# pflanze/LAPIS-SILO

Hardware: AMD Instinct MI355X
Metric: Mutations-scan positions*sequences/s (higher is better)
Workload: dtype u64; 1 GPU; 10000000-sequence x 29903-nt nucleotide Mutations scan (minProportion 0.05) with a PangoLineage sublineage filter (B.1*), through QueryEngine::executeQuery; sequences=10000000, positions=29903, mutation_rows=412

## Files before the change

include/silo_gpu.h:

```cpp
#ifndef SILO_GPU_H
#define SILO_GPU_H

#include <stddef.h>
#include <stdint.h>

#ifdef __cplusplus
extern "C" {
#endif

typedef enum {
   SILO_GPU_OK = 0,
   SILO_GPU_ERR_INVALID_ARGUMENT = -1,
   SILO_GPU_ERR_OUT_OF_MEMORY = -2,
   SILO_GPU_ERR_HIP = -3,
   SILO_GPU_ERR_NO_DEVICE = -4,
   SILO_GPU_ERR_PROGRAM_TOO_LARGE = -5,
   SILO_GPU_ERR_UNSUPPORTED = -6
} silo_gpu_status;

enum { SILO_GPU_ALPHABET_NUCLEOTIDE = 0, SILO_GPU_ALPHABET_AMINO_ACID = 1 };
enum { SILO_GPU_NUC_SYMBOLS = 16, SILO_GPU_AA_SYMBOLS = 25, SILO_GPU_MAX_SYMBOLS = 25 };
#define SILO_GPU_SYMBOL_NONE 0xFFu

typedef struct silo_gpu_store silo_gpu_store;
// ... 182 lines not shown
);
int silo_gpu_reconstruct_sequences(
   const silo_gpu_store* store, uint32_t seqstore_id, const uint32_t* row_ids_dev, uint32_t n_rows, char* out_chars_dev, void* stream
);

typedef struct silo_gpu_mutation_row {
   uint32_t position;
   uint32_t symbol_index;
   uint32_t count;
   uint32_t total;
} silo_gpu_mutation_row;
int silo_gpu_mutations_select(
   const uint32_t* counts_dev, const uint8_t* reference_index_dev, uint32_t n_positions, uint32_t n_symbols, double min_proportion,
   uint32_t capacity, uint32_t* out_dev, void* stream
);
typedef struct silo_gpu_row_slot silo_gpu_row_slot;
int silo_gpu_row_slot_create(uint32_t row_capacity, silo_gpu_row_slot** out_slot);
void silo_gpu_row_slot_destroy(silo_gpu_row_slot* slot);
int silo_gpu_mutations_select_to_slot(
   const uint32_t* counts_dev, const uint8_t* reference_index_dev, uint32_t n_positions, uint32_t n_symbols, double min_proportion,
   silo_gpu_row_slot* slot, void* stream
);
int silo_gpu_row_slot_wait(silo_gpu_row_slot* slot, const silo_gpu_mutation_row** out_rows, uint32_t* out_selected, void* stream);
int silo_gpu_upload_bytes(const void* src_host, size_t bytes, void** out_dev);

int silo_gpu_mutations_scan(
   const silo_gpu_store* store, uint32_t seqstore_id, const uint64_t* filter_dev,
   uint32_t pos_begin, uint32_t pos_end, uint32_t* counts_out_dev, void* stream
);
uint32_t silo_gpu_store_scan_planes(const silo_gpu_store* store, uint32_t seqstore_id);
uint64_t silo_gpu_store_scan_escapes(const silo_gpu_store* store, uint32_t seqstore_id);
uint64_t silo_gpu_store_scan_overflow_keys(const silo_gpu_store* store, uint32_t seqstore_id);
uint64_t silo_gpu_store_scan_rows(const silo_gpu_store* store, uint32_t seqstore_id, uint32_t pos_begin, uint32_t pos_end);
uint64_t silo_gpu_store_scan_runs(const silo_gpu_store* store, uint32_t seqstore_id);
uint64_t silo_gpu_store_scan_sparse_keys(const silo_gpu_store* store, uint32_t seqstore_id);
int silo_gpu_store_finalize_seqstore(silo_gpu_store* store, uint32_t seqstore_id);

typedef struct silo_gpu_scan_range {
   uint32_t seqstore_id;
   uint32_t pos_begin;
   uint32_t pos_end;
} silo_gpu_scan_range;
int silo_gpu_mutations_scan_ranges(
   const silo_gpu_store* store, const silo_gpu_scan_range* ranges, uint32_t n_ranges, const uint64_t* const* filters_dev, uint32_t n_filters,
   uint32_t* const* counts_out_dev, void* stream
);

int silo_gpu_mutations_scan_ranges_min_proportion(
   const silo_gpu_store* store, const silo_gpu_scan_range* ranges, uint32_t n_ranges, const uint64_t* const* filters_dev, uint32_t n_filters,
   const double* min_proportion , uint32_t* const* counts_out_dev, void* stream
);
typedef struct silo_gpu_select_sink {
   uint32_t* table_dev;
   uint32_t total_positions;
   uint32_t n_symbols;
   const uint8_t* reference_index_dev;
   silo_gpu_row_slot* slot;
} silo_gpu_select_sink;
int silo_gpu_mutations_scan_select(
   const silo_gpu_store* store, const silo_gpu_scan_range* ranges, uint32_t n_ranges, const uint64_t* const* filters_dev, uint32_t n_filters,
   const double* min_proportion , uint32_t* const* counts_out_dev, const silo_gpu_select_sink* sinks , void* stream
);
int silo_gpu_store_scan_prunable_granules(
   const silo_gpu_store* store, uint32_t seqstore_id, uint32_t cardinality, double min_proportion, uint64_t* out_skippable, uint64_t* out_total
);
int silo_gpu_store_scan_prunable_rows(
   const silo_gpu_store* store, uint32_t seqstore_id, uint32_t cardinality, double min_proportion, uint64_t* out_skippable, uint64_t* out_total
);
uint64_t silo_gpu_store_scan_covered_rows(const silo_gpu_store* store, uint32_t seqstore_id);
uint64_t silo_gpu_store_scan_end_events(const silo_gpu_store* store, uint32_t seqstore_id);
uint64_t silo_gpu_store_scan_residual_keys(const silo_gpu_store* store, uint32_t seqstore_id);

#define SILO_GPU_MAX_DATE_RANGES 1024
#define SILO_GPU_MAX_GROUPED_MUTATIONS 4096
#define SILO_GPU_GROUPED_SCRATCH_BYTES(row_words, n_ranges, n_mutations)                                                    \
   ((size_t)(row_words) * 128u + (size_t)(n_mutations) * 32u + (size_t)(n_ranges) * 16u +                                   \
    (size_t)(n_ranges) * 4u * (1u + 3u * (size_t)(n_mutations)) + 1024u)
int silo_gpu_mutations_grouped(
   const silo_gpu_store* store, uint32_t seqstore_id, const uint64_t* filter_dev, const uint32_t* date_column_dev, const uint32_t* range_bounds,
   uint32_t n_ranges, const uint32_t* positions, const uint32_t* symbols, uint32_t n_mutations, void* group_scratch_dev, uint32_t* out_dev,
   void* stream
);

#define SILO_GPU_MAX_GROUPED_FILTERS 2048
#define SILO_GPU_FILTERS_GROUPED_SCRATCH_BYTES(row_words, n_ranges, n_filters)                                              \
   ((size_t)(row_words) * 128u + (size_t)(n_filters) * 8u + (size_t)(n_ranges) * 16u + 1024u)
int silo_gpu_filters_grouped(
   const silo_gpu_store* store, const uint64_t* base_filter_dev, const uint32_t* date_column_dev, const uint32_t* range_bounds, uint32_t n_ranges,
   const uint64_t* const* filters_dev, uint32_t n_filters, void* scratch_dev, uint32_t* out_dev, void* stream
);

#define SILO_GPU_MAX_CROSS_FILTERS 1024
#define SILO_GPU_CROSS_TILE 8
#define SILO_GPU_CROSS_CHUNK_WORDS 1024
#define SILO_GPU_FILTERS_CROSS_SCRATCH_BYTES(n_rows, n_cols) (((size_t)(n_rows) + (size_t)(n_cols)) * 16u + 1024u)
int silo_gpu_filters_cross(
   const silo_gpu_store* store, const uint64_t* base_filter_dev, const uint64_t* const* row_filters_dev, const uint32_t* row_index, uint32_t n_rows,
   const uint64_t* const* col_filters_dev, const uint32_t* col_index, uint32_t n_cols, void* scratch_dev, uint32_t* out_dev, uint32_t out_rows,
   uint32_t out_cols, void* stream
);

#define SILO_GPU_MAX_DISTANCE_ROWS 2048
#define SILO_GPU_DISTANCE_PLANES(alphabet) ((alphabet) == SILO_GPU_ALPHABET_AMINO_ACID ? 6u : 4u)
#define SILO_GPU_DISTANCE_WORDS(positions) (((positions) + 63u) / 64u)
#define SILO_GPU_DISTANCE_TILE 16
#define SILO_GPU_DISTANCE_CHUNK_WORDS 32
int silo_gpu_distance_pack(int alphabet, const char* chars_dev, uint32_t n_rows, uint32_t positions, uint64_t* planes_dev, void* stream);
int silo_gpu_distance_pairs(int alphabet, const uint64_t* planes_dev, uint32_t n_rows, uint32_t positions, uint32_t* out_dev, void* stream);

#define SILO_GPU_MAX_CLUSTER_ROWS 8192
#define SILO_GPU_ADJACENCY_WORDS(n_rows) (((n_rows) + 63u) / 64u)
#define SILO_GPU_WITHIN_TILE_ROWS 16
#define SILO_GPU_WITHIN_TILE_COLS 64
#define SILO_GPU_WITHIN_CHUNK_WORDS 16
#define SILO_GPU_COMPONENTS_THREADS 1024
int silo_gpu_distance_within(
   int alphabet, const uint64_t* planes_dev, uint32_t n_rows, uint32_t positions, uint32_t max_distance, uint32_t min_compared,
   uint64_t* adjacency_dev, void* stream
);
int silo_gpu_adjacency_components(const uint64_t* adjacency_dev, uint32_t n_rows, uint32_t* labels_dev, uint32_t* rounds_dev, void* stream);

#define SILO_GPU_MAX_SPANNING_ROWS 8192
#define SILO_GPU_SPANNING_THREADS 1024
#define SILO_GPU_SPANNING_KEY_ROW_BITS 13
#define SILO_GPU_SPANNING_KEY_WEIGHT_SHIFT 26
#define SILO_GPU_SPANNING_KEY(weight, i, j) \
   (((uint64_t)(weight) << SILO_GPU_SPANNING_KEY_WEIGHT_SHIFT) | ((uint64_t)(i) << SILO_GPU_SPANNING_KEY_ROW_BITS) | (uint64_t)(j))
int silo_gpu_distance_weights(
   int alphabet, const uint64_t* planes_dev, uint32_t n_rows, uint32_t positions, uint32_t max_distance, uint32_t min_compared,
   uint32_t* weights_dev, void* stream
);
int silo_gpu_spanning_forest(const uint32_t* weights_dev, uint32_t n_rows, uint64_t* edges_dev, uint32_t* count_dev, void* stream);
int silo_gpu_distance_listed_pairs(
   int alphabet, const uint64_t* planes_dev, uint32_t n_rows, uint32_t positions, const uint64_t* edges_dev, const uint32_t* count_dev,
   uint32_t max_pairs, uint32_t* out_dev, void* stream
);

#define SILO_GPU_MAX_CROSS_ROWS 2048
#define SILO_GPU_MAX_CROSS_COLUMNS 8192
#define SILO_GPU_MAX_NEIGHBOUR_COLUMNS 64
#define SILO_GPU_NEIGHBOUR_THREADS 1024
#define SILO_GPU_NEIGHBOUR_KEY_COLUMN_BITS 13
int silo_gpu_distance_cross(
   int alphabet, const uint64_t* row_planes_dev, uint32_t n_rows, const uint64_t* column_planes_dev, uint32_t n_columns, uint32_t positions,
   const uint32_t* self_column_dev, uint32_t max_distance, uint32_t min_compared, uint32_t* cells_dev, void* stream
);
int silo_gpu_nearest_columns(
   const uint32_t* cells_dev, uint32_t n_rows, uint32_t n_columns, uint32_t k, uint32_t* out_dev, uint32_t* counts_dev, void* stream
);

#define SILO_GPU_MAX_CONSENSUS_TABLES 64
#define SILO_GPU_CONSENSUS_THREADS 256
int silo_gpu_consensus_call(
   int alphabet, const uint32_t* counts_dev, uint32_t n_tables, uint32_t n_positions, const uint8_t* reference_index_dev, double threshold,
   uint32_t min_depth, char* out_chars_dev, uint32_t* out_summary_dev, void* stream
);

#define SILO_GPU_MAX_HAPLOTYPE_POSITIONS 12
#define SILO_GPU_HAPLOTYPE_POSITIONS_PER_COLUMN 6
int silo_gpu_position_symbols(
   const silo_gpu_store* store, uint32_t seqstore_id, const uint32_t* positions , uint32_t n_positions,
   uint8_t* out_symbols_dev , uint32_t* out_unresolved_dev , void* stream
);
int silo_gpu_haplotype_ids(
   const uint8_t* symbols_dev, uint32_t n_positions, uint32_t row_words, uint32_t sequence_count, uint32_t n_symbols,
   uint32_t complete_symbols , const uint64_t* filter_dev ,
   uint32_t* const* out_ids_dev , uint64_t* out_rows_dev ,
   void* stream
);

#define SILO_GPU_MAX_COMPARISON_TABLES 64
#define SILO_GPU_COMPARE_THREADS 256
int silo_gpu_mutations_compare(
   int alphabet, const uint32_t* counts_dev, uint32_t n_tables, uint32_t n_positions, const uint8_t* reference_index_dev, double min_proportion,
   double min_difference, uint32_t capacity, uint32_t* out_dev, void* stream
);

#define SILO_GPU_MAX_DIFFERENCE_ROWS 10000
#define SILO_GPU_MAX_DIFFERENCE_POSITIONS (1u << 23)
#define SILO_GPU_DIFFERENCE_STATS 4
#define SILO_GPU_DIFFERENCE_CHUNK 4096
#define SILO_GPU_DIFFERENCE_CHUNKS(positions) (((positions) + 15u + SILO_GPU_DIFFERENCE_CHUNK - 1u) / SILO_GPU_DIFFERENCE_CHUNK)
#define SILO_GPU_DIFFERENCES_SCRATCH_BYTES(n_rows, positions) \
   ((size_t)(n_rows) * SILO_GPU_DIFFERENCE_CHUNKS(positions) * (1u + SILO_GPU_DIFFERENCE_STATS) * sizeof(uint32_t))
int silo_gpu_sequence_differences(
   int alphabet, const char* chars_dev , uint32_t n_rows, uint32_t positions, const char* reference_dev ,
   uint32_t capacity, uint32_t* offsets_dev , uint32_t* stats_dev ,
   uint32_t* records_dev , void* scratch_dev, void* stream
);

#define SILO_GPU_MAX_NEAREST_ROWS 1024
#define SILO_GPU_QUERY_DISTANCE_COUNTER_PLANES 12
#define SILO_GPU_QUERY_DISTANCE_SCRATCH_BYTES(positions)                                                                    \
   (((size_t)(positions) / 256u + 1u) * 256u + 2u * ((((size_t)(positions) + 1u) * 4u) / 256u + 1u) * 256u)
#define SILO_GPU_NEAREST_ROWS_SCRATCH_BYTES 32768u
int silo_gpu_query_distances(
   const silo_gpu_store* store, uint32_t seqstore_id, const char* query_chars, uint32_t* out_dev, void* scratch_dev, void* stream
);
int silo_gpu_nearest_rows(
   const uint32_t* table_dev, const uint64_t* filter_dev, uint32_t sequence_count, uint32_t exclude_row, uint32_t max_distance, uint32_t k,
   uint32_t* out_dev, uint32_t* out_count_dev, void* scratch_dev, void* stream
);
int silo_gpu_bitset_from_distances(
   const uint32_t* table_dev, uint32_t sequence_count, uint32_t row_words, uint32_t max_distance, uint32_t min_compared, uint64_t* out_bitset_dev,
   void* stream
);

#define SILO_GPU_MAX_SAMPLE_GROUPS 1024
#define SILO_GPU_SAMPLE_LDS_GROUPS 16
#define SILO_GPU_SAMPLE_ROUNDS 4
#define SILO_GPU_SAMPLE_STATE_BYTES(n_groups) (16u + (size_t)(n_groups) * (16u + 256u * 4u))
uint32_t silo_gpu_sample_key(uint64_t seed, uint32_t global_row);
int silo_gpu_sample_groups(
   const uint64_t* filter_dev, const uint32_t* date_column_dev, const uint32_t* range_bounds, uint32_t n_ranges, uint32_t sequence_count,
   uint32_t row_words, uint16_t* groups_out_dev, void* stream
);
int silo_gpu_sample_begin(void* state_dev, uint32_t n_groups, uint32_t size, uint64_t seed, void* stream);
int silo_gpu_sample_count(
   void* state_dev, const uint64_t* filter_dev, const uint16_t* groups_dev, uint32_t sequence_count, uint32_t row_words, uint32_t first_row,
   uint32_t round, void* stream
);
int silo_gpu_sample_advance(void* state_dev, uint32_t round, void* stream);
int silo_gpu_sample_select(
   const void* state_dev, const uint64_t* filter_dev, const uint16_t* groups_dev, uint32_t sequence_count, uint32_t row_words,
   uint32_t first_row, uint64_t* out_bitset_dev, void* stream
);

#define SILO_GPU_ROW_HASH_NO_SYMBOL 31u
#define SILO_GPU_ROW_HASH_SCRATCH_BYTES(positions) ((size_t)(positions) * 17u + 1024u)
#define SILO_GPU_DISTINCT_EMPTY 0xFFFFFFFFu
#define SILO_GPU_DISTINCT_TABLE_BYTES(slots) (((size_t)(slots) + 1u) * 4u)
typedef struct silo_gpu_distinct_part {
   const uint64_t* hashes_dev;
   uint32_t first_row;
   uint32_t sequence_count;
   uint32_t row_words;
   uint32_t reserved;
} silo_gpu_distinct_part;
uint64_t silo_gpu_row_hash_term(uint32_t position, uint32_t symbol, uint32_t lane);
int silo_gpu_row_hashes(const silo_gpu_store* store, uint32_t seqstore_id, uint64_t* out_dev, void* scratch_dev, void* stream);
int silo_gpu_store_row_hashes(silo_gpu_store* store, uint32_t seqstore_id, const uint64_t** out_dev, void* stream);
int silo_gpu_distinct_begin(void* table_dev, uint32_t slots, void* stream);
int silo_gpu_distinct_insert(
   void* table_dev, uint32_t slots, const silo_gpu_distinct_part* parts_dev, uint32_t n_parts, uint32_t part, const uint64_t* filter_dev,
   void* stream
);
int silo_gpu_distinct_select(
   const void* table_dev, uint32_t slots, const silo_gpu_distinct_part* parts_dev, uint32_t n_parts, uint32_t part,
   const uint64_t* filter_dev, uint64_t* out_bitset_dev, void* stream
);

#define SILO_GPU_MAX_DISTINCT_CLASSES 16384
#define SILO_GPU_DISTINCT_COUNTS_BYTES(slots) ((size_t)(slots) * 4u)
#define SILO_GPU_SMALLEST_KEYS_SCRATCH_BYTES 1088u
int silo_gpu_distinct_count(
   void* table_dev, uint32_t slots, uint32_t* counts_dev, const silo_gpu_distinct_part* parts_dev, uint32_t n_parts, uint32_t part,
   const uint64_t* filter_dev, void* stream
);
int silo_gpu_distinct_classes(
   void* table_dev, uint32_t slots, const uint32_t* counts_dev, const silo_gpu_distinct_part* parts_dev, uint32_t n_parts, uint32_t part,
   const uint64_t* filter_dev, uint32_t min_count, uint64_t* keys_dev, uint32_t capacity, uint32_t* n_keys_dev, void* stream
);
int silo_gpu_smallest_keys(
   const uint64_t* keys_dev, const uint32_t* n_keys_dev, uint32_t capacity, uint32_t k, uint64_t* out_dev, uint32_t* out_count_dev, void* scratch_dev,
   void* stream
);

#define SILO_GPU_CELL_COUNT_KINDS 4
#define SILO_GPU_CELL_COUNT_SUBSTITUTIONS 1u
#define SILO_GPU_CELL_COUNT_DELETIONS 2u
#define SILO_GPU_CELL_COUNT_MISSING 4u
#define SILO_GPU_CELL_COUNT_AMBIGUOUS 8u
#define SILO_GPU_MAX_CELL_COUNT_BINS 4096
#define SILO_GPU_ROW_CELL_COUNT_SCRATCH_BYTES(positions) ((size_t)(positions) * 17u + 1024u)
int silo_gpu_row_cell_counts(const silo_gpu_store* store, uint32_t seqstore_id, uint32_t* out_dev, void* scratch_dev, void* stream);
int silo_gpu_store_row_cell_counts(silo_gpu_store* store, uint32_t seqstore_id, const uint32_t** out_dev, void* stream);
int silo_gpu_bitset_from_cell_counts(
   const uint32_t* table_dev, uint32_t row_words, uint32_t sequence_count, uint32_t kinds_mask, uint32_t at_least, uint32_t at_most,
   uint64_t* out_bitset_dev, void* stream
);
int silo_gpu_cell_count_histogram(
   const uint32_t* table_dev, uint32_t row_words, uint32_t sequence_count, const uint64_t* filter_dev, uint32_t kinds_mask, uint32_t bin_width,
   uint32_t n_bins, uint64_t* bins_dev, void* stream
);

enum { SILO_GPU_MAX_SCAN_BATCH = 8 };
int silo_gpu_mutations_scan_batch(
   const silo_gpu_store* store, uint32_t seqstore_id, const uint64_t* const* filters_dev, uint32_t n_filters,
   uint32_t pos_begin, uint32_t pos_end, uint32_t* const* counts_out_dev, void* stream
);
int silo_gpu_memset_async(void* dev_ptr, int value, size_t bytes, void* stream);

enum { SILO_GPU_TUNE_SCAN_ROWS_PER_BLOCK = 0, SILO_GPU_TUNE_SCAN_VARIANT = 1, SILO_GPU_TUNE_EVAL_LEAF_BATCH = 2 ,
       SILO_GPU_TUNE_COMPACT_INDEX = 4 ,
       SILO_GPU_TUNE_KEY_COST = 6 ,
       SILO_GPU_TUNE_MISSING_RUNS = 8 ,
       SILO_GPU_TUNE_LAUNCH_COST = 9 ,
       SILO_GPU_TUNE_SCAN_TIMING = 7 ,
       SILO_GPU_TUNE_SIDE_STREAM = 5 ,
       SILO_GPU_TUNE_GAP_EVENTS = 10 ,
       SILO_GPU_TUNE_PRUNE_KEYS = 11 ,
       SILO_GPU_TUNE_END_RUNS = 12 ,
       SILO_GPU_TUNE_FUSED_SELECT = 13 ,
       SILO_GPU_TUNE_SCAN_SPARSE_DIVISOR = 3  };
int silo_gpu_tune(int knob, int value);

int silo_gpu_event_create(void** out_event);
int silo_gpu_event_record(void* event, void* stream);
int silo_gpu_event_synchronize(void* event);
int silo_gpu_event_elapsed_ms(void* start_event, void* stop_event, float* out_ms);
void silo_gpu_event_destroy(void* event);

typedef struct silo_gpu_comm silo_gpu_comm;
enum { SILO_GPU_COMM_ID_BYTES = 128 };
int silo_gpu_comm_unique_id(uint8_t* out_id );
int silo_gpu_comm_create(const uint8_t* id, uint32_t rank, uint32_t world, int device, silo_gpu_comm** out);
void silo_gpu_comm_destroy(silo_gpu_comm* comm);
uint32_t silo_gpu_comm_rank(const silo_gpu_comm* comm);
uint32_t silo_gpu_comm_world(const silo_gpu_comm* comm);
int silo_gpu_allreduce_counts(silo_gpu_comm* comm, uint32_t* counts_dev, size_t n, void* stream);
int silo_gpu_broadcast_bytes(silo_gpu_comm* comm, void* bytes_dev, size_t n_bytes, uint32_t root, void* stream);

const char* silo_gpu_last_scan_kernel(void);

typedef struct silo_gpu_scan_timing {
   char kernel[64];
   uint64_t plane_rows;
   uint64_t bytes;
   uint32_t filters;
   uint32_t blocks;
   float ms;
} silo_gpu_scan_timing;
int silo_gpu_scan_timings(silo_gpu_scan_timing* out, uint32_t capacity, uint32_t* n_out);

int silo_gpu_stream_read_probe(uint64_t bytes, uint32_t reps, float* out_ms_per_pass);

const char* silo_gpu_last_error(void);

#ifdef __cplusplus
}
#endif
#endif
```

lapis-silo_amd/csrc/scan_internal.h:

```cpp
#pragma once
#include <stdint.h>

#include <algorithm>
#include <array>
#include <vector>

#include "store_internal.h"

namespace silo_gpu_detail {

constexpr uint32_t SCAN_MAX_RANGES = 32;
constexpr uint32_t SPARSE_COUNTER_STRIDE = 64;
constexpr uint32_t SECTOR_WORDS = 8;
constexpr uint32_t COMPACT_THREADS = 1024;
constexpr uint32_t ROW_LIST_MAX = 1024;

__device__ __forceinline__ bool takesGatherScan(const uint32_t* __restrict__ counters, uint32_t capacity) {
   const uint32_t sectors = counters[0];
   return sectors <= capacity && static_cast<uint64_t>(sectors) * 8u < static_cast<uint64_t>(counters[1]) * (COMPACT_THREADS / SECTOR_WORDS) * 5u;
}

struct ScanBatchArgs {
   const uint64_t* filters[SILO_GPU_MAX_SCAN_BATCH];
   const uint32_t* sparse_sectors;
   uint32_t sparse_capacity;
   uint32_t n_ranges;
   const uint64_t* planes[SCAN_MAX_RANGES];
   uint32_t n_positions[SCAN_MAX_RANGES];
   uint32_t first_unit[SCAN_MAX_RANGES + 1];
   uint32_t* counts[SCAN_MAX_RANGES][SILO_GPU_MAX_SCAN_BATCH];
   const uint8_t* code_map[SCAN_MAX_RANGES];
   uint32_t target_base[SCAN_MAX_RANGES];
   uint32_t out_symbols;
   const uint8_t* row_covered[SCAN_MAX_RANGES];
};

enum : int { KIND_IDENTITY = 0, KIND_MAPPED = 1, KIND_ROWS = 2 };

struct RowPruneArgs {
   const uint32_t* counters;
   double min_proportion[SILO_GPU_MAX_SCAN_BATCH];
   const uint32_t* heaviest[SCAN_MAX_RANGES];
   const uint32_t* without[SCAN_MAX_RANGES];
};
static_assert(sizeof(ScanBatchArgs) + sizeof(RowPruneArgs) + 3 * sizeof(uint32_t) <= 4096, "k_scan_sliced takes its arguments by value: the kernel-argument segment holds 4 KiB");

inline void copyFilters(const uint64_t* (&dst)[SILO_GPU_MAX_SCAN_BATCH], const uint64_t* const* filters, uint32_t n) {
   std::copy_n(filters, n, dst);
}

struct ScanPiece {
   const uint64_t* planes;
   const uint8_t* code_map;
   uint32_t n_positions;
   uint32_t target_base;
   const uint32_t* row_heaviest;
   const uint32_t* row_without;
   const uint8_t* row_covered;
   uint32_t* counts[SILO_GPU_MAX_SCAN_BATCH];
};

enum ScanLayout { SCAN_2_PLANES = 0, SCAN_3_PLANES_MAPPED, SCAN_FULL_NUCLEOTIDE, SCAN_FULL_AMINO_ACID, SCAN_ONE_HOT_ROWS, N_SCAN_LAYOUTS };

constexpr uint32_t DERIVED_MAX_RANGES = 16;

struct DerivedRange {
   uint32_t* scratch;
   uint32_t stride;
   uint32_t n_positions;
   uint32_t n_scan;
   uint32_t pos_begin;
   uint32_t gaps_offset;
   uint32_t ends_offset;
   uint32_t table_offset;
   const uint8_t* code_map;
   const uint8_t* position_covered;
   uint32_t end_symbol;
   const uint64_t* run_keys;
   const uint32_t* run_ends;
   const uint32_t* run_slice_first;
   const uint64_t* sparse_keys;
   uint32_t sparse_begin;
   uint32_t sparse_end;
   uint32_t* caller_counts[SILO_GPU_MAX_SCAN_BATCH];
};
struct SelectSink {
   const uint8_t* reference_index;
   uint32_t* cursor_and_ticket;
   silo_gpu_mutation_row* host_rows;
   unsigned long long* host_header;
   double min_proportion;
   uint32_t capacity;
   uint32_t epoch;
   uint32_t total_blocks;
};
struct DerivedArgs {
   const uint64_t* filters[SILO_GPU_MAX_SCAN_BATCH];
   const uint32_t* counters;
   uint32_t row_words;
   uint32_t n_run_slices;
   uint32_t n_ranges;
   uint32_t first_unit[DERIVED_MAX_RANGES + 1];
   uint32_t* run_parts;
   uint32_t* run_flags;
   uint32_t part_stride;
   uint32_t run_blocks_per_slice;
   DerivedRange ranges[DERIVED_MAX_RANGES];
   SelectSink sinks[SILO_GPU_MAX_SCAN_BATCH];
};
static_assert(sizeof(DerivedArgs) <= 4096, "the kernels of the derived symbols take their arguments by value: the kernel-argument segment holds 4 KiB");

struct DerivedPlan {
   std::vector<DerivedArgs> launches;
   std::vector<ScanRange> private_ranges;
   bool events = false;
   std::vector<ScanRange> gap_ranges;
   std::vector<uint8_t> end_runs;
   std::vector<ScanRange> end_ranges;
   bool ends_apart = false;
   std::vector<std::array<uint64_t, DERIVED_MAX_RANGES>> run_counts;
   size_t table_words = 0;
   size_t part_words = 0;
   uint32_t most_positions = 0;
   bool select = false;
};

struct ScanSelect {
   SelectSink sinks[SILO_GPU_MAX_SCAN_BATCH];
   std::vector<uint32_t> table_offset;
};

struct ScanPruning {
   const uint32_t* counters;
   const double* min_proportion;
   bool keys;
   bool rows;
};

struct ScanLaunchTiming;
ScanLaunchTiming* startLaunchTiming(const char* kernel, uint64_t plane_rows, uint64_t bytes, uint32_t filters, uint32_t blocks, hipStream_t stream);
void finishLaunchTiming(ScanLaunchTiming* timing, hipStream_t stream);

int scanShortRows(const std::vector<ScanRange>& ranges, bool nucleotide, const uint64_t* const* filters, uint32_t q_count, hipStream_t hip_stream);
hipError_t prepareScan(const uint64_t* const* filters, uint32_t q_count,
   uint32_t row_words, uint32_t capacity, uint32_t* counters, uint32_t* sector_index, uint32_t* tables, uint32_t table_words, uint32_t* counters_to_reset, hipStream_t hip_stream);
int scanPiecesDense(const std::vector<ScanPiece> (&pieces)[N_SCAN_LAYOUTS], const SeqStoreDev& any_store, const uint64_t* const* filters, uint32_t q_count,
   const uint32_t* sparse_sectors, uint32_t sparse_capacity, hipStream_t hip_stream, const ScanPruning* pruning);
int scanPiecesGather(const std::vector<ScanPiece> (&pieces)[N_SCAN_LAYOUTS], const SeqStoreDev& any_store, const uint64_t* const* filters, uint32_t q_count,
   const uint32_t* sparse_sectors, uint32_t sparse_capacity, const uint32_t* sector_index, uint32_t stride, hipStream_t hip_stream);

int scanEscapes(const std::vector<ScanRange>& ranges, const uint64_t* const* filters, uint32_t q_count, hipStream_t hip_stream, const std::vector<ScanRange>* gaps, const ScanPruning* pruning,
   const std::vector<ScanRange>* ends = nullptr, bool only_ends = false);

bool derivedCountsEvents(const std::vector<ScanRange>& ranges);
void planDerived(const silo_gpu_store* store, const std::vector<ScanRange>& ranges, const uint64_t* const* filters, uint32_t q_count, DerivedPlan& plan,
   const ScanSelect* select = nullptr);
void bindDerived(DerivedPlan& plan, uint32_t* tables, const uint32_t* counters, uint32_t q_count);
int scanRowsWithoutSymbol(DerivedPlan& plan, uint32_t q_count, hipStream_t hip_stream);
int finishDerived(DerivedPlan& plan, uint32_t q_count, hipStream_t hip_stream);

}
```

lapis-silo_amd/csrc/silo_gpu_runtime.hip:

```cpp
#include <hip/hip_runtime.h>

#include <stdint.h>
#include <stdio.h>
#include <string.h>

#include <algorithm>
#include <array>
#include <atomic>
#include <memory>
#include <mutex>
#include <new>
#include <string>
#include <vector>

#include "store_internal.h"

std::atomic<int> g_tune_rows_per_block{0};
std::atomic<int> g_tune_scan_variant{0};
std::atomic<int> g_tune_eval_leaf_batch{0};
std::atomic<int> g_tune_compact_index{0};
std::atomic<int> g_tune_side_stream{0};
std::atomic<int> g_tune_scan_timing{0};
std::atomic<int> g_tune_missing_runs{0};
std::atomic<int> g_tune_key_cost{0};
std::atomic<int> g_tune_launch_cost{0};
std::atomic<int> g_tune_sparse_divisor{0};
std::atomic<int> g_tune_gap_events{0};
std::atomic<int> g_tune_prune_keys{0};
std::atomic<int> g_tune_end_runs{0};
std::atomic<int> g_tune_fused_select{0};

namespace {
thread_local std::string g_last_error;
}

int silo_gpu_internal_fail(int code, const std::string& message) {
   g_last_error = message;
   return code;
}

using namespace silo_gpu_detail;

extern "C" {

const char* silo_gpu_last_error(void) {
   return g_last_error.c_str();
}

int silo_gpu_tune(int knob, int value) {
   if (knob == SILO_GPU_TUNE_SCAN_ROWS_PER_BLOCK) {
      return g_tune_rows_per_block.exchange(value);
   }
   if (knob == SILO_GPU_TUNE_SCAN_VARIANT) {
      return g_tune_scan_variant.exchange(value);
   }
   if (knob == SILO_GPU_TUNE_EVAL_LEAF_BATCH) {
      return g_tune_eval_leaf_batch.exchange(value);
   }
   if (knob == SILO_GPU_TUNE_SCAN_SPARSE_DIVISOR) {
      return g_tune_sparse_divisor.exchange(value);
   }
   if (knob == SILO_GPU_TUNE_COMPACT_INDEX) {
      return g_tune_compact_index.exchange(value);
   }
   if (knob == SILO_GPU_TUNE_SIDE_STREAM) {
      return g_tune_side_stream.exchange(value);
   }
   if (knob == SILO_GPU_TUNE_KEY_COST) {
      return g_tune_key_cost.exchange(value);
   }
   if (knob == SILO_GPU_TUNE_SCAN_TIMING) {
      return g_tune_scan_timing.exchange(value);
   }
   if (knob == SILO_GPU_TUNE_MISSING_RUNS) {
      return g_tune_missing_runs.exchange(value);
   }
   if (knob == SILO_GPU_TUNE_LAUNCH_COST) {
      return g_tune_launch_cost.exchange(value);
   }
   if (knob == SILO_GPU_TUNE_GAP_EVENTS) {
      return g_tune_gap_events.exchange(value);
   }
   if (knob == SILO_GPU_TUNE_PRUNE_KEYS) {
      return g_tune_prune_keys.exchange(value);
   }
   if (knob == SILO_GPU_TUNE_END_RUNS) {
      return g_tune_end_runs.exchange(value);
   }
   if (knob == SILO_GPU_TUNE_FUSED_SELECT) {
      return g_tune_fused_select.exchange(value);
   }
   return -1;
}

int silo_gpu_malloc(size_t bytes, void** out_dev) {
   if (out_dev == nullptr) {
      return fail(SILO_GPU_ERR_INVALID_ARGUMENT, "silo_gpu_malloc: null out pointer");
   }
   HIP_TRY(hipMalloc(out_dev, bytes));
   return SILO_GPU_OK;
}

void silo_gpu_free(void* dev_ptr) {
   (void)hipFree(dev_ptr);
}


int silo_gpu_memset_async(void* dev_ptr, int value, size_t bytes, void* stream) {
   HIP_TRY(hipMemsetAsync(dev_ptr, value, bytes, static_cast<hipStream_t>(stream)));
   return SILO_GPU_OK;
}

int silo_gpu_memcpy_d2h(void* dst_host, const void* src_dev, size_t bytes, void* stream) {
   constexpr size_t PINNED_BYTES = 4u << 20;
   struct Pinned {
      void* ptr = nullptr;
      bool tried = false;
   };
   thread_local Pinned pinned;
   if (bytes <= PINNED_BYTES && !pinned.tried) {
      pinned.tried = true;
      if (hipHostMalloc(&pinned.ptr, PINNED_BYTES, hipHostMallocDefault) != hipSuccess) {
         (void)hipGetLastError();
         pinned.ptr = nullptr;
      }
   }
   auto hip_stream = static_cast<hipStream_t>(stream);
   if (bytes <= PINNED_BYTES && pinned.ptr != nullptr) {
      HIP_TRY(hipMemcpyAsync(pinned.ptr, src_dev, bytes, hipMemcpyDeviceToHost, hip_stream));
      HIP_TRY(hipStreamSynchronize(hip_stream));
      memcpy(dst_host, pinned.ptr, bytes);
      return SILO_GPU_OK;
   }
   HIP_TRY(hipMemcpyAsync(dst_host, src_dev, bytes, hipMemcpyDeviceToHost, hip_stream));
   HIP_TRY(hipStreamSynchronize(hip_stream));
   return SILO_GPU_OK;
}

int silo_gpu_host_alloc(size_t bytes, void** out_host) {
   if (out_host == nullptr || bytes == 0) {
      return fail(SILO_GPU_ERR_INVALID_ARGUMENT, "silo_gpu_host_alloc: bad arguments");
   }
   HIP_TRY(hipHostMalloc(out_host, bytes, hipHostMallocDefault));
   return SILO_GPU_OK;
}

void silo_gpu_host_free(void* host) {
   if (host != nullptr) {
      (void)hipHostFree(host);
   }
}

int silo_gpu_memcpy_d2h_async(void* dst_pinned_host, const void* src_dev, size_t bytes, void* stream) {
   if (dst_pinned_host == nullptr || src_dev == nullptr) {
      return fail(SILO_GPU_ERR_INVALID_ARGUMENT, "silo_gpu_memcpy_d2h_async: null pointer");
   }
   HIP_TRY(hipMemcpyAsync(dst_pinned_host, src_dev, bytes, hipMemcpyDeviceToHost, static_cast<hipStream_t>(stream)));
   return SILO_GPU_OK;
}

int silo_gpu_memcpy_h2d(void* dst_dev, const void* src_host, size_t bytes, void* stream) {
   HIP_TRY(hipMemcpyAsync(dst_dev, src_host, bytes, hipMemcpyHostToDevice, static_cast<hipStream_t>(stream)));
   HIP_TRY(hipStreamSynchronize(static_cast<hipStream_t>(stream)));
   return SILO_GPU_OK;
}

int silo_gpu_event_create(void** out_event) {
   if (out_event == nullptr) {
      return fail(SILO_GPU_ERR_INVALID_ARGUMENT, "silo_gpu_event_create: null out pointer");
   }
   hipEvent_t event = nullptr;
   HIP_TRY(hipEventCreate(&event));
   *out_event = event;
   return SILO_GPU_OK;
}

int silo_gpu_event_synchronize(void* event) {
   HIP_TRY(hipEventSynchronize(static_cast<hipEvent_t>(event)));
   return SILO_GPU_OK;
}

int silo_gpu_event_record(void* event, void* stream) {
   HIP_TRY(hipEventRecord(static_cast<hipEvent_t>(event), static_cast<hipStream_t>(stream)));
   return SILO_GPU_OK;
}

int silo_gpu_event_elapsed_ms(void* start_event, void* stop_event, float* out_ms) {
   HIP_TRY(hipEventSynchronize(static_cast<hipEvent_t>(stop_event)));
   HIP_TRY(hipEventElapsedTime(out_ms, static_cast<hipEvent_t>(start_event), static_cast<hipEvent_t>(stop_event)));
   return SILO_GPU_OK;
}

void silo_gpu_event_destroy(void* event) {
   (void)hipEventDestroy(static_cast<hipEvent_t>(event));
}

int silo_gpu_set_device(int device) {
   HIP_TRY(hipSetDevice(device));
   return SILO_GPU_OK;
}

int silo_gpu_stream_create(void** out_stream) {
   if (out_stream == nullptr) {
      return fail(SILO_GPU_ERR_INVALID_ARGUMENT, "silo_gpu_stream_create: null out pointer");
   }
   hipStream_t stream = nullptr;
   HIP_TRY(hipStreamCreateWithFlags(&stream, hipStreamNonBlocking));
   *out_stream = stream;
   return SILO_GPU_OK;
}

void silo_gpu_stream_destroy(void* stream) {
   if (stream != nullptr) {
      (void)hipStreamDestroy(static_cast<hipStream_t>(stream));
   }
}

int silo_gpu_stream_synchronize(void* stream) {
   HIP_TRY(hipStreamSynchronize(static_cast<hipStream_t>(stream)));
   return SILO_GPU_OK;
}


namespace {
__global__ __launch_bounds__(256) void k_stream_sum(const uint64_t* __restrict__ data, uint64_t n_chunks, unsigned long long* __restrict__ sink) {
   constexpr uint32_t IN_FLIGHT = 16;
   const uint64_t per_block = (n_chunks + gridDim.x - 1) / gridDim.x;
   const uint64_t begin = static_cast<uint64_t>(blockIdx.x) * per_block;
   const uint64_t end = min(n_chunks, begin + per_block);
   uint64_t sum = 0;
   for (uint64_t base = begin; base < end; base += 256u * IN_FLIGHT) {
      ulonglong2 value[IN_FLIGHT];
#pragma unroll
      for (uint32_t k = 0; k < IN_FLIGHT; ++k) {
         const uint64_t chunk = base + k * 256u + threadIdx.x;
         value[k] = chunk < end ? loadPlane16<true>(data + chunk * 2u) : make_ulonglong2(0, 0);
      }
#pragma unroll
      for (uint32_t k = 0; k < IN_FLIGHT; ++k) {
         sum += value[k].x + value[k].y;
      }
   }
   if (sum == 0x123456789ABCDEFull) {
      atomicAdd(sink, 1ull);
   }
}
}

int silo_gpu_stream_read_probe(uint64_t bytes, uint32_t reps, float* out_ms_per_pass) {
   if (out_ms_per_pass == nullptr || bytes < (1u << 20) || reps == 0) {
      return fail(SILO_GPU_ERR_INVALID_ARGUMENT, "silo_gpu_stream_read_probe: bad arguments");
   }
   DeviceArray<uint64_t> data;
   DeviceArray<unsigned long long> sink;
   hipEvent_t start = nullptr, stop = nullptr;
   bytes &= ~uint64_t{15};
   hipError_t status = data.alloc(bytes / sizeof(uint64_t));
   status = status != hipSuccess ? status : sink.alloc(1);
   status = status != hipSuccess ? status : hipMemset(data.get(), 0x5A, bytes);
   status = status != hipSuccess ? status : hipMemset(sink.get(), 0, sizeof(unsigned long long));
   status = status != hipSuccess ? status : hipEventCreate(&start);
   status = status != hipSuccess ? status : hipEventCreate(&stop);
   float ms = 0;
   if (status == hipSuccess) {
      const uint32_t blocks = 256u * 32u;
      k_stream_sum<<<blocks, 256>>>(data.get(), bytes / 16, sink.get());
      status = hipEventRecord(start, nullptr);
      for (uint32_t rep = 0; rep < reps && status == hipSuccess; ++rep) {
         k_stream_sum<<<blocks, 256>>>(data.get(), bytes / 16, sink.get());
         status = hipGetLastError();
      }
      status = status != hipSuccess ? status : hipEventRecord(stop, nullptr);
      status = status != hipSuccess ? status : hipEventSynchronize(stop);
      status = status != hipSuccess ? status : hipEventElapsedTime(&ms, start, stop);
   }
   if (start != nullptr) {
      (void)hipEventDestroy(start);
   }
   if (stop != nullptr) {
      (void)hipEventDestroy(stop);
   }
   HIP_TRY(status);
   *out_ms_per_pass = ms / static_cast<float>(reps);
   return SILO_GPU_OK;
}

int silo_gpu_upload_bytes(const void* src_host, size_t bytes, void** out_dev) {
   if (src_host == nullptr || out_dev == nullptr || bytes == 0) {
      return fail(SILO_GPU_ERR_INVALID_ARGUMENT, "silo_gpu_upload_bytes: bad arguments");
   }
   DeviceArray<uint8_t> dev;
   HIP_TRY(dev.alloc(bytes));
   const hipError_t status = hipMemcpy(dev.get(), src_host, bytes, hipMemcpyHostToDevice);
   HIP_TRY(status);
   *out_dev = dev.release();
   return SILO_GPU_OK;
}

int silo_gpu_upload_u32(const uint32_t* src_host, size_t n, uint32_t** out_dev) {
   if (out_dev == nullptr || (src_host == nullptr && n > 0)) {
      return fail(SILO_GPU_ERR_INVALID_ARGUMENT, "silo_gpu_upload_u32: bad arguments");
   }
   DeviceArray<uint32_t> dev;
   HIP_TRY(dev.alloc(std::max<size_t>(n, 1)));
   hipError_t err = hipMemcpy(dev.get(), src_host, n * sizeof(uint32_t), hipMemcpyHostToDevice);
   if (err != hipSuccess) {
      return fail(SILO_GPU_ERR_HIP, std::string("silo_gpu_upload_u32: ") + hipGetErrorString(err));
   }
   *out_dev = dev.release();
   return SILO_GPU_OK;
}

}
```

lapis-silo_amd/csrc/silo_gpu_scan.hip:

```cpp
#include <hip/hip_runtime.h>

#include <stdint.h>
#include <stdio.h>

#include <algorithm>
#include <memory>
#include <mutex>
#include <string>
#include <vector>

#include "fused_select_rule.h"
#include "scan_internal.h"

using namespace silo_gpu_detail;

namespace {

thread_local const char* g_last_scan_kernel = "none";

__global__ void k_add_u32(uint32_t* __restrict__ dst, const uint32_t* __restrict__ src, uint32_t n) {
   const uint32_t i = blockIdx.x * blockDim.x + threadIdx.x;
   if (i < n) {
      dst[i] += src[i];
   }
// ... 184 lines not shown
SideStreams* sideStreams() {
   thread_local SideStreams side;
   if (!side.tried) {
      side.tried = true;
      side.ok = true;
      int least = 0, greatest = 0;
      (void)hipDeviceGetStreamPriorityRange(&least, &greatest);
      for (int k = 0; k < N_SIDE_STREAMS; ++k) {
         side.ok = side.ok && hipStreamCreateWithPriority(&side.stream[k], hipStreamNonBlocking, k == 0 ? least : 0) == hipSuccess &&
                   hipEventCreateWithFlags(&side.join[k], hipEventDisableTiming) == hipSuccess;
      }
      for (int k = 0; k < 2; ++k) {
         side.ok = side.ok && hipEventCreateWithFlags(&side.fork[k], hipEventDisableTiming) == hipSuccess;
      }
      if (!side.ok) {
         (void)hipGetLastError();
      }
   }
   return side.ok ? &side : nullptr;
}

int forkSide(SideStreams* side, int k, int fork_index, hipStream_t hip_stream, bool record) {
   if (record) {
      HIP_TRY(hipEventRecord(side->fork[fork_index], hip_stream));
   }
   HIP_TRY(hipStreamWaitEvent(side->stream[k], side->fork[fork_index], 0));
   side->used[k] = true;
   return SILO_GPU_OK;
}

int joinSides(hipStream_t hip_stream) {
   SideStreams* side = sideStreams();
   if (side == nullptr) {
      return SILO_GPU_OK;
   }
   for (int k = 0; k < N_SIDE_STREAMS; ++k) {
      if (side->used[k]) {
         side->used[k] = false;
         HIP_TRY(hipEventRecord(side->join[k], side->stream[k]));
         HIP_TRY(hipStreamWaitEvent(hip_stream, side->join[k], 0));
      }
   }
   return SILO_GPU_OK;
}

int forkSidePasses(
   const std::vector<ScanRange>& ranges, const uint64_t* const* filters, uint32_t q_count, DerivedPlan* derived, hipStream_t hip_stream,
   const ScanPruning* pruning
) {
   bool any_escapes = false;
   for (const ScanRange& range : ranges) {
      const SeqStoreHost::Layout& layout = range.seqstore->layout;
      any_escapes = any_escapes || (layout.built && layout.d_escapes.get() != nullptr && layout.escape_first[range.pos_end] != layout.escape_first[range.pos_begin]);
   }
   if (!any_escapes && derived == nullptr) {
      return SILO_GPU_OK;
   }
   if (derived != nullptr && derived->events) {
      return scanEscapes(ranges, filters, q_count, hip_stream, &derived->gap_ranges, pruning, derived->ends_apart ? nullptr : &derived->end_ranges);
   }
   const int mode = g_tune_side_stream.load();
   SideStreams* side = mode == 2 ? nullptr : sideStreams();
   hipStream_t stream = hip_stream;
   if (side != nullptr) {
      const int k = mode == 1 || derived != nullptr ? 1 : 0;
      if (const int rc = forkSide(side, k, 0, hip_stream, true); rc != SILO_GPU_OK) {
         return rc;
      }
      stream = side->stream[k];
   }
   if (derived != nullptr) {
      if (const int rc = scanRowsWithoutSymbol(*derived, q_count, stream); rc != SILO_GPU_OK) {
         return rc;
      }
      return any_escapes ? scanEscapes(ranges, filters, q_count, mode == 1 ? stream : hip_stream, nullptr, nullptr) : SILO_GPU_OK;
   }
   return scanEscapes(ranges, filters, q_count, stream, nullptr, nullptr);
}

}

int silo_gpu_detail::scanRanges(
   const silo_gpu_store* store, const std::vector<ScanRange>& caller_ranges, const uint64_t* const* filters, uint32_t q_count, hipStream_t hip_stream,
   const double* min_proportion, const ScanSelect* select
) {
   const SeqStoreDev& any_store = caller_ranges.front().seqstore->dev;
   const bool nucleotide = any_store.n_bits == 3 && any_store.n_scan == 5;
   if (!nucleotide && !(any_store.n_bits == 5 && any_store.n_scan == 22)) {
      return fail(SILO_GPU_ERR_INVALID_ARGUMENT, "mutations scan: unsupported set of scan symbols (5 nucleotide or 22 amino-acid symbols)");
   }
   if (any_store.row_words < SCAN_THREADS * 4) {
      if (select != nullptr) {
         return fail(SILO_GPU_ERR_INVALID_ARGUMENT, "mutations scan: short rows do not go through the finish kernel");
      }
      const int rc = scanShortRows(caller_ranges, nucleotide, filters, q_count, hip_stream);
      if (rc == SILO_GPU_OK) {
         g_last_scan_kernel = "k_scan_sliced_rowwave";
      }
      return rc;
   }
   g_last_scan_kernel = q_count == 1 ? "k_scan_sliced" : "k_scan_sliced_batch";
   scanTimingLog().used = 0;
   bool any_derived = false;
   for (const ScanRange& range : caller_ranges) {
      any_derived = any_derived || range.seqstore->layout.has_implicit;
   }
   DerivedPlan plan;
   if (any_derived) {
      planDerived(store, caller_ranges, filters, q_count, plan, select);
   }
   if (select != nullptr && !plan.select) {
      return fail(SILO_GPU_ERR_INVALID_ARGUMENT, "mutations scan: this scan cannot select its rows in the finish kernel");
   }
   const int divisor = g_tune_sparse_divisor.load();
   const bool routing = divisor >= 0;
   if (!routing && !any_derived) {
      std::vector<ScanPiece> pieces[N_SCAN_LAYOUTS];
      cutIntoPieces(caller_ranges, q_count, pieces, nullptr);
      int rc = forkSidePasses(caller_ranges, filters, q_count, nullptr, hip_stream, nullptr);
      if (rc == SILO_GPU_OK) {
         rc = scanPiecesDense(pieces, any_store, filters, q_count, nullptr, 0, hip_stream, nullptr);
      }
      const int joined = joinSides(hip_stream);
      return rc != SILO_GPU_OK ? rc : joined;
   }
   const uint32_t capacity = std::max<uint32_t>(4, any_store.row_words / static_cast<uint32_t>(divisor <= 0 ? 16 : divisor));
   SparseScratch* scratch = nullptr;
   const int acquired = acquireSparseScratch(store->device, capacity, plan.table_words + plan.part_words, &scratch);
   if (acquired != SILO_GPU_OK) {
      return acquired;
   }
   const uint32_t stride = scratch->capacity;
   uint32_t* counters = scratch->counters[scratch->set];
   if (any_derived) {
      bindDerived(plan, scratch->tables, counters, q_count);
   }
   const std::vector<ScanRange>& ranges = any_derived ? plan.private_ranges : caller_ranges;
   std::vector<ScanPiece> pieces[N_SCAN_LAYOUTS];
   cutIntoPieces(ranges, q_count, pieces, any_derived ? &plan.end_runs : nullptr);
   bool some_proportion = false;
   for (uint32_t q = 0; min_proportion != nullptr && q < q_count; ++q) {
      some_proportion = some_proportion || (min_proportion[q] > 0 && min_proportion[q] <= 1);
   }
   const int prune_knob = g_tune_prune_keys.load();
   const bool prune_keys = some_proportion && plan.events && prune_knob >= 0;
   const ScanPruning pruning{counters, min_proportion, prune_keys, prune_keys && prune_knob == 0};
   const ScanPruning* pruned = pruning.keys ? &pruning : nullptr;
   if (prepareScan(filters, q_count, any_store.row_words, stride, counters, scratch->sector_index, scratch->tables, static_cast<uint32_t>(plan.table_words),
                   scratch->counters[scratch->set ^ 1u], hip_stream) != hipSuccess) {
      scratch->set ^= 1u;
      releaseSparseScratch(scratch, hip_stream);
      return fail(SILO_GPU_ERR_HIP, "mutations scan: the prepare step could not be launched");
   }
   int rc = forkSidePasses(ranges, filters, q_count, any_derived ? &plan : nullptr, hip_stream, pruned);
   if (rc == SILO_GPU_OK) {
      rc = scanPiecesDense(pieces, any_store, filters, q_count, routing ? counters : nullptr, capacity, hip_stream, pruned);
   }
   if (rc == SILO_GPU_OK && any_derived && plan.events && plan.ends_apart) {
      rc = scanEscapes(ranges, filters, q_count, hip_stream, &plan.gap_ranges, nullptr, &plan.end_ranges, true);
   }
   if (rc == SILO_GPU_OK && routing) {
      rc = scanPiecesGather(pieces, any_store, filters, q_count, counters, capacity, scratch->sector_index, stride, hip_stream);
   }
   const int joined = joinSides(hip_stream);
   if (rc == SILO_GPU_OK && joined == SILO_GPU_OK && any_derived) {
      rc = finishDerived(plan, q_count, hip_stream);
   }
   releaseSparseScratch(scratch, hip_stream);
   return rc != SILO_GPU_OK ? rc : joined;
}

static bool canFuseSelect(
   const silo_gpu_store* store, const silo_gpu_scan_range* ranges, uint32_t n_ranges, uint32_t n_filters, uint32_t* const* counts_out_dev,
   const silo_gpu_select_sink* sinks, std::vector<uint32_t>& table_offset
) {
   if (g_tune_fused_select.load() < 0 || n_ranges == 0 || n_filters == 0) {
      return false;
   }
   const uint32_t n_symbols = sinks[0].n_symbols;
   if (n_symbols != 5 && n_symbols != 22) {
      return false;
   }
   std::vector<ScanRange> group;
   std::vector<TableSpan> spans;
   bool any_derived = false;
   table_offset.assign(n_ranges, 0);
   for (uint32_t r = 0; r < n_ranges; ++r) {
      const SeqStoreHost& seqstore = store->seqstores[ranges[r].seqstore_id];
      const uint32_t n = ranges[r].pos_end - ranges[r].pos_begin;
      if (n == 0) {
         continue;
      }
      if (seqstore.dev.n_scan != n_symbols || seqstore.dev.planes == nullptr || seqstore.dev.row_words < static_cast<uint32_t>(SCAN_THREADS) * 4) {
         return false;
      }
      any_derived = any_derived || seqstore.layout.has_implicit;
      group.push_back(ScanRange{&seqstore, ranges[r].pos_begin, ranges[r].pos_end, {}});
      for (uint32_t q = 0; q < n_filters; ++q) {
         const silo_gpu_select_sink& sink = sinks[q];
         const uint32_t* at = counts_out_dev[static_cast<size_t>(r) * n_filters + q];
         if (sink.n_symbols != n_symbols || sink.total_positions != sinks[0].total_positions || at < sink.table_dev) {
            return false;
         }
         const size_t words = static_cast<size_t>(at - sink.table_dev);
         if (words % n_symbols != 0 || words / n_symbols >= sink.total_positions) {
            return false;
         }
         const auto offset = static_cast<uint32_t>(words / n_symbols);
         if (q != 0 && offset != table_offset[r]) {
            return false;
         }
         table_offset[r] = offset;
      }
      spans.push_back({table_offset[r], n});
   }
   return any_derived && derivedCountsEvents(group) && spansTileTable(spans, sinks[0].total_positions);
}

static int scanRangesEntry(
   const char* entry, const silo_gpu_store* store, const silo_gpu_scan_range* ranges, uint32_t n_ranges, const uint64_t* const* filters_dev, uint32_t n_filters,
   const double* min_proportion, uint32_t* const* counts_out_dev, void* stream, const silo_gpu_select_sink* sinks = nullptr,
   const std::vector<uint32_t>* table_offset = nullptr
) {
   if (store == nullptr || (n_ranges != 0 && ranges == nullptr) || (n_filters != 0 && filters_dev == nullptr) ||
       (n_ranges != 0 && n_filters != 0 && counts_out_dev == nullptr)) {
      return fail(SILO_GPU_ERR_INVALID_ARGUMENT, std::string(entry) + ": bad arguments");
   }
   for (uint32_t q = 0; q < n_filters; ++q) {
      if (filters_dev[q] == nullptr) {
         return fail(SILO_GPU_ERR_INVALID_ARGUMENT, std::string(entry) + ": null filter");
      }
   }
   for (uint32_t r = 0; r < n_ranges; ++r) {
      if (ranges[r].seqstore_id >= store->seqstores.size()) {
         return fail(SILO_GPU_ERR_INVALID_ARGUMENT, std::string(entry) + ": no such sequence store");
      }
      const SeqStoreDev& dev = store->seqstores[ranges[r].seqstore_id].dev;
      if (ranges[r].pos_begin > ranges[r].pos_end || ranges[r].pos_end > dev.positions) {
         return fail(SILO_GPU_ERR_INVALID_ARGUMENT, "position range out of bounds");
      }
      for (uint32_t q = 0; q < n_filters; ++q) {
         if (counts_out_dev[static_cast<size_t>(r) * n_filters + q] == nullptr) {
            return fail(SILO_GPU_ERR_INVALID_ARGUMENT, std::string(entry) + ": null counts buffer");
         }
      }
   }
   if (n_ranges == 0 || n_filters == 0) {
      return SILO_GPU_OK;
   }
   HIP_TRY(hipSetDevice(store->device));
   auto hip_stream = static_cast<hipStream_t>(stream);
   for (uint32_t first = 0; first < n_filters; first += SILO_GPU_MAX_SCAN_BATCH) {
      const uint32_t q_count = std::min<uint32_t>(SILO_GPU_MAX_SCAN_BATCH, n_filters - first);
      for (const uint32_t n_bits : {3u, 5u}) {
         std::vector<ScanRange> group;
         ScanSelect select;
         for (uint32_t r = 0; r < n_ranges; ++r) {
            const SeqStoreDev& dev = store->seqstores[ranges[r].seqstore_id].dev;
            if (ranges[r].pos_begin == ranges[r].pos_end || dev.n_scan == 0 || (dev.n_bits == 3 ? 3u : 5u) != n_bits) {
               continue;
            }
            const SeqStoreHost& seqstore = store->seqstores[ranges[r].seqstore_id];
            if (dev.planes == nullptr) {
               return fail(SILO_GPU_ERR_INVALID_ARGUMENT, std::string(entry) + ": the sequence store holds no sequences yet");
            }
            ScanRange range{&seqstore, ranges[r].pos_begin, ranges[r].pos_end, {}};
            for (uint32_t q = 0; q < q_count; ++q) {
               range.counts[q] = counts_out_dev[static_cast<size_t>(r) * n_filters + first + q];
            }
            group.push_back(range);
            if (sinks != nullptr) {
               select.table_offset.push_back((*table_offset)[r]);
            }
         }
         for (uint32_t q = 0; sinks != nullptr && !group.empty() && q < q_count; ++q) {
            const silo_gpu_select_sink& sink = sinks[first + q];
            silo_gpu_row_slot* slot = sink.slot;
            slot->epoch += 1;
            if (slot->epoch == 0) {
               slot->epoch = 1;
            }
            select.sinks[q] = SelectSink{
               sink.reference_index_dev, slot->d_cursor_and_ticket.get(), reinterpret_cast<silo_gpu_mutation_row*>(static_cast<char*>(slot->host_dev) + 16),
               static_cast<unsigned long long*>(slot->host_dev), min_proportion != nullptr ? min_proportion[first + q] : 0.0, slot->capacity, slot->epoch, 0};
         }
         if (!group.empty()) {
            const int rc = scanRanges(store, group, filters_dev + first, q_count, hip_stream, min_proportion != nullptr ? min_proportion + first : nullptr,
                                      sinks != nullptr ? &select : nullptr);
            if (rc != SILO_GPU_OK) {
               return rc;
            }
         }
      }
   }
   return SILO_GPU_OK;
}

extern "C" {

const char* silo_gpu_last_scan_kernel(void) {
   return g_last_scan_kernel;
}

int silo_gpu_mutations_scan_ranges(
   const silo_gpu_store* store, const silo_gpu_scan_range* ranges, uint32_t n_ranges, const uint64_t* const* filters_dev, uint32_t n_filters,
   uint32_t* const* counts_out_dev, void* stream
) {
   return scanRangesEntry("silo_gpu_mutations_scan_ranges", store, ranges, n_ranges, filters_dev, n_filters, nullptr, counts_out_dev, stream);
}

int silo_gpu_mutations_scan_ranges_min_proportion(
   const silo_gpu_store* store, const silo_gpu_scan_range* ranges, uint32_t n_ranges, const uint64_t* const* filters_dev, uint32_t n_filters,
   const double* min_proportion, uint32_t* const* counts_out_dev, void* stream
) {
   return scanRangesEntry("silo_gpu_mutations_scan_ranges_min_proportion", store, ranges, n_ranges, filters_dev, n_filters, min_proportion, counts_out_dev, stream);
}

int silo_gpu_mutations_scan_select(
   const silo_gpu_store* store, const silo_gpu_scan_range* ranges, uint32_t n_ranges, const uint64_t* const* filters_dev, uint32_t n_filters,
   const double* min_proportion, uint32_t* const* counts_out_dev, const silo_gpu_select_sink* sinks, void* stream
) {
   const char* entry = "silo_gpu_mutations_scan_select";
   if (store == nullptr || sinks == nullptr || n_filters == 0 || filters_dev == nullptr || n_ranges == 0 || ranges == nullptr || counts_out_dev == nullptr) {
      return fail(SILO_GPU_ERR_INVALID_ARGUMENT, std::string(entry) + ": bad arguments");
   }
   for (uint32_t q = 0; q < n_filters; ++q) {
      const silo_gpu_select_sink& sink = sinks[q];
      if (filters_dev[q] == nullptr || sink.table_dev == nullptr || sink.reference_index_dev == nullptr || sink.slot == nullptr || sink.total_positions == 0 ||
          sink.n_symbols == 0 || sink.n_symbols > 32) {
         return fail(SILO_GPU_ERR_INVALID_ARGUMENT, std::string(entry) + ": bad filter or sink");
      }
      for (uint32_t other = 0; other < q; ++other) {
         if (sinks[other].slot == sink.slot || sinks[other].table_dev == sink.table_dev) {
            return fail(SILO_GPU_ERR_INVALID_ARGUMENT, std::string(entry) + ": two filters share a table or a row slot");
         }
      }
   }
   for (uint32_t r = 0; r < n_ranges; ++r) {
      if (ranges[r].seqstore_id >= store->seqstores.size()) {
         return fail(SILO_GPU_ERR_INVALID_ARGUMENT, std::string(entry) + ": no such sequence store");
      }
      if (ranges[r].pos_begin > ranges[r].pos_end || ranges[r].pos_end > store->seqstores[ranges[r].seqstore_id].dev.positions) {
         return fail(SILO_GPU_ERR_INVALID_ARGUMENT, "position range out of bounds");
      }
      for (uint32_t q = 0; q < n_filters; ++q) {
         if (counts_out_dev[static_cast<size_t>(r) * n_filters + q] == nullptr) {
            return fail(SILO_GPU_ERR_INVALID_ARGUMENT, std::string(entry) + ": null counts buffer");
         }
      }
   }
   std::vector<uint32_t> table_offset;
   if (canFuseSelect(store, ranges, n_ranges, n_filters, counts_out_dev, sinks, table_offset)) {
      return scanRangesEntry(entry, store, ranges, n_ranges, filters_dev, n_filters, min_proportion, counts_out_dev, stream, sinks, &table_offset);
   }
   HIP_TRY(hipSetDevice(store->device));
   for (uint32_t q = 0; q < n_filters; ++q) {
      HIP_TRY(hipMemsetAsync(sinks[q].table_dev, 0, static_cast<size_t>(sinks[q].total_positions) * sinks[q].n_symbols * sizeof(uint32_t), static_cast<hipStream_t>(stream)));
   }
   if (const int rc = scanRangesEntry(entry, store, ranges, n_ranges, filters_dev, n_filters, min_proportion, counts_out_dev, stream); rc != SILO_GPU_OK) {
      return rc;
   }
   for (uint32_t q = 0; q < n_filters; ++q) {
      const int rc = silo_gpu_mutations_select_to_slot(
         sinks[q].table_dev, sinks[q].reference_index_dev, sinks[q].total_positions, sinks[q].n_symbols, min_proportion != nullptr ? min_proportion[q] : 0.0,
         sinks[q].slot, stream
      );
      if (rc != SILO_GPU_OK) {
         return rc;
      }
   }
   return SILO_GPU_OK;
}

int silo_gpu_scan_timings(silo_gpu_scan_timing* out, uint32_t capacity, uint32_t* n_out) {
   if (n_out == nullptr || (capacity != 0 && out == nullptr)) {
      return fail(SILO_GPU_ERR_INVALID_ARGUMENT, "silo_gpu_scan_timings: bad arguments");
   }
   ScanTimingLog& log = scanTimingLog();
   *n_out = static_cast<uint32_t>(log.used);
   for (size_t k = 0; k < log.used && k < capacity; ++k) {
      ScanLaunchTiming& launch = log.launches[k];
      HIP_TRY(hipEventSynchronize(launch.stop));
      HIP_TRY(hipEventElapsedTime(&launch.entry.ms, launch.start, launch.stop));
      out[k] = launch.entry;
   }
   return SILO_GPU_OK;
}

int silo_gpu_mutations_scan_batch(
   const silo_gpu_store* store, uint32_t seqstore_id, const uint64_t* const* filters_dev, uint32_t n_filters, uint32_t pos_begin,
   uint32_t pos_end, uint32_t* const* counts_out_dev, void* stream
) {
   if (store == nullptr || seqstore_id >= store->seqstores.size() || filters_dev == nullptr || counts_out_dev == nullptr) {
      return fail(SILO_GPU_ERR_INVALID_ARGUMENT, "silo_gpu_mutations_scan_batch: bad arguments");
   }
   const silo_gpu_scan_range range{seqstore_id, pos_begin, pos_end};
   return silo_gpu_mutations_scan_ranges(store, &range, 1, filters_dev, n_filters, counts_out_dev, stream);
}

uint32_t silo_gpu_store_scan_planes(const silo_gpu_store* store, uint32_t seqstore_id) {
   if (store == nullptr || seqstore_id >= store->seqstores.size()) {
      return 0;
   }
   const SeqStoreHost& seqstore = store->seqstores[seqstore_id];
   uint64_t positions_with[8] = {0, 0, 0, 0, 0, 0, 0, 0};
   for (const SeqStoreHost::Run& run : seqstore.layout.runs) {
      for (uint32_t p = run.begin; run.one_hot && p < run.end; ++p) {
         positions_with[(seqstore.layout.row_of[p + 1] - seqstore.layout.row_of[p]) & 7u] += 1;
      }
      positions_with[run.bits & 7u] += run.one_hot ? 0 : run.end - run.begin;
   }
   uint32_t most_common = seqstore.dev.n_bits;
   uint64_t most = 0;
   for (uint32_t bits = 0; bits < 8; ++bits) {
      if (positions_with[bits] > most) {
         most = positions_with[bits];
         most_common = bits;
      }
   }
   return most_common;
}

uint64_t silo_gpu_store_scan_rows(const silo_gpu_store* store, uint32_t seqstore_id, uint32_t pos_begin, uint32_t pos_end) {
   if (store == nullptr || seqstore_id >= store->seqstores.size()) {
      return 0;
   }
   const SeqStoreHost& seqstore = store->seqstores[seqstore_id];
   pos_end = std::min(pos_end, seqstore.dev.positions);
   if (pos_begin >= pos_end) {
      return 0;
   }
   if (seqstore.layout.row_of.empty()) {
      return static_cast<uint64_t>(pos_end - pos_begin) * seqstore.dev.n_bits;
   }
   return seqstore.layout.row_of[pos_end] - seqstore.layout.row_of[pos_begin];
}

uint64_t silo_gpu_store_scan_runs(const silo_gpu_store* store, uint32_t seqstore_id) {
   if (store == nullptr || seqstore_id >= store->seqstores.size() || !store->seqstores[seqstore_id].layout.has_implicit) {
      return 0;
   }
   return store->seqstores[seqstore_id].dev.n_missing_runs;
}

uint64_t silo_gpu_store_scan_sparse_keys(const silo_gpu_store* store, uint32_t seqstore_id) {
   if (store == nullptr || seqstore_id >= store->seqstores.size() || !store->seqstores[seqstore_id].layout.has_implicit) {
      return 0;
   }
   return store->seqstores[seqstore_id].sparse_sorted.size();
}

int silo_gpu_store_scan_prunable_granules(
   const silo_gpu_store* store, uint32_t seqstore_id, uint32_t cardinality, double min_proportion, uint64_t* out_skippable, uint64_t* out_total
) {
   if (store == nullptr || seqstore_id >= store->seqstores.size() || out_skippable == nullptr || out_total == nullptr) {
      return fail(SILO_GPU_ERR_INVALID_ARGUMENT, "silo_gpu_store_scan_prunable_granules: bad arguments");
   }
   const SeqStoreHost::Layout& layout = store->seqstores[seqstore_id].layout;
   *out_total = layout.escapes_sliced.packed_keys / ESCAPE_GRANULE_KEYS;
   *out_skippable = 0;
   for (size_t g = 0; g < layout.granule_heaviest.size(); ++g) {
      *out_skippable += granulePrunable(cardinality, layout.granule_without[g], layout.granule_heaviest[g], min_proportion) ? 1 : 0;
   }
   return SILO_GPU_OK;
}

int silo_gpu_store_scan_prunable_rows(
   const silo_gpu_store* store, uint32_t seqstore_id, uint32_t cardinality, double min_proportion, uint64_t* out_skippable, uint64_t* out_total
) {
   if (store == nullptr || seqstore_id >= store->seqstores.size() || out_skippable == nullptr || out_total == nullptr) {
      return fail(SILO_GPU_ERR_INVALID_ARGUMENT, "silo_gpu_store_scan_prunable_rows: bad arguments");
   }
   const SeqStoreHost::Layout& layout = store->seqstores[seqstore_id].layout;
   *out_total = 0;
   *out_skippable = 0;
   for (const SeqStoreHost::Run& run : layout.runs) {
      for (uint32_t row = run.one_hot ? layout.row_of[run.begin] : 0; run.one_hot && row < layout.row_of[run.end]; ++row) {
         *out_total += 1;
         if (row < layout.row_heaviest.size()) {
            *out_skippable += granulePrunable(cardinality, layout.row_without[row], layout.row_heaviest[row], min_proportion) ? 1 : 0;
         }
      }
   }
   return SILO_GPU_OK;
}

uint64_t silo_gpu_store_scan_covered_rows(const silo_gpu_store* store, uint32_t seqstore_id) {
   return store == nullptr || seqstore_id >= store->seqstores.size() ? 0 : store->seqstores[seqstore_id].layout.covered_rows;
}

uint64_t silo_gpu_store_scan_end_events(const silo_gpu_store* store, uint32_t seqstore_id) {
   return store == nullptr || seqstore_id >= store->seqstores.size() ? 0 : store->seqstores[seqstore_id].layout.end_events;
}

uint64_t silo_gpu_store_scan_residual_keys(const silo_gpu_store* store, uint32_t seqstore_id) {
   return store == nullptr || seqstore_id >= store->seqstores.size() ? 0 : store->seqstores[seqstore_id].layout.residual_keys;
}

uint64_t silo_gpu_store_scan_escapes(const silo_gpu_store* store, uint32_t seqstore_id) {
   if (store == nullptr || seqstore_id >= store->seqstores.size() || store->seqstores[seqstore_id].layout.escape_first.empty()) {
      return 0;
   }
   return store->seqstores[seqstore_id].layout.escape_first.back();
}

uint64_t silo_gpu_store_scan_overflow_keys(const silo_gpu_store* store, uint32_t seqstore_id) {
   if (store == nullptr || seqstore_id >= store->seqstores.size() || !store->seqstores[seqstore_id].layout.built) {
      return 0;
   }
   return store->seqstores[seqstore_id].layout.escapes_sliced.n_overflow;
}


int silo_gpu_mutations_scan(
   const silo_gpu_store* store, uint32_t seqstore_id, const uint64_t* filter_dev, uint32_t pos_begin, uint32_t pos_end,
   uint32_t* counts_out_dev, void* stream
) {
   if (store == nullptr || seqstore_id >= store->seqstores.size() || counts_out_dev == nullptr) {
      return fail(SILO_GPU_ERR_INVALID_ARGUMENT, "silo_gpu_mutations_scan: bad arguments");
   }
   HIP_TRY(hipSetDevice(store->device));
   const SeqStoreDev& dev = store->seqstores[seqstore_id].dev;
   if (pos_begin > pos_end || pos_end > dev.positions) {
      return fail(SILO_GPU_ERR_INVALID_ARGUMENT, "position range out of bounds");
   }
   if (pos_begin == pos_end || dev.n_scan == 0) {
      return SILO_GPU_OK;
   }
   auto hip_stream_early = static_cast<hipStream_t>(stream);
   if (filter_dev == nullptr) {
      auto* mutable_store = const_cast<silo_gpu_store*>(store);
      SeqStoreHost& seqstore = mutable_store->seqstores[seqstore_id];
      const size_t n_totals = static_cast<size_t>(dev.positions) * dev.n_scan;
      {
         const std::lock_guard<std::mutex> lock(mutable_store->mutex);
         if (!seqstore.totals_ready) {
            if (seqstore.d_totals.get() == nullptr) {
               HIP_TRY(seqstore.d_totals.alloc(n_totals));
            }
            HIP_TRY(hipMemsetAsync(seqstore.d_totals.get(), 0, n_totals * sizeof(uint32_t), hip_stream_early));
            const int rc = silo_gpu_mutations_scan(store, seqstore_id, store->d_ones.get(), 0, dev.positions, seqstore.d_totals.get(), stream);
            if (rc != SILO_GPU_OK) {
               return rc;
            }
            HIP_TRY(hipStreamSynchronize(hip_stream_early));
            seqstore.totals_ready = true;
         }
      }
      const uint32_t n = (pos_end - pos_begin) * dev.n_scan;
      k_add_u32<<<(n + 255) / 256, 256, 0, hip_stream_early>>>(
         counts_out_dev, seqstore.d_totals.get() + static_cast<size_t>(pos_begin) * dev.n_scan, n
      );
      HIP_TRY(hipGetLastError());
      g_last_scan_kernel = "k_add_u32 (cached totals)";
      return SILO_GPU_OK;
   }
   const silo_gpu_scan_range range{seqstore_id, pos_begin, pos_end};
   return silo_gpu_mutations_scan_ranges(store, &range, 1, &filter_dev, 1, &counts_out_dev, stream);
}



}
```

lapis-silo_amd/csrc/silo_gpu_scan_keys.hip:

```cpp
#include <hip/hip_runtime.h>

#include <stdint.h>
#include <stdio.h>

#include <algorithm>
#include <array>
#include <mutex>
#include <string>
#include <type_traits>
#include <vector>

#include "scan_internal.h"

using namespace silo_gpu_detail;

namespace {

constexpr uint32_t ESCAPE_KEYS_PER_THREAD = 4;
__global__ __launch_bounds__(256) void k_scan_escapes(
   const uint64_t* __restrict__ escapes, uint32_t n_escapes, const ScanBatchArgs batch, uint32_t pos_begin
) {
   const uint32_t q = blockIdx.y;
   const uint32_t lane = threadIdx.x & 63u;
   const uint32_t first = blockIdx.x * (256u * ESCAPE_KEYS_PER_THREAD) + threadIdx.x;
   uint64_t key[ESCAPE_KEYS_PER_THREAD];
   bool selected[ESCAPE_KEYS_PER_THREAD];
#pragma unroll
   for (uint32_t k = 0; k < ESCAPE_KEYS_PER_THREAD; ++k) {
      const uint32_t i = first + k * 256u;
      key[k] = i < n_escapes ? escapes[i] : 0;
   }
#pragma unroll
   for (uint32_t k = 0; k < ESCAPE_KEYS_PER_THREAD; ++k) {
      const uint32_t sequence = static_cast<uint32_t>(key[k]);
      selected[k] = first + k * 256u < n_escapes && ((batch.filters[q][sequence >> 6] >> (sequence & 63u)) & 1ull) != 0;
   }
#pragma unroll
   for (uint32_t k = 0; k < ESCAPE_KEYS_PER_THREAD; ++k) {
      bool pending = selected[k];
      const uint32_t counter = (static_cast<uint32_t>(key[k] >> 37) - pos_begin) * batch.out_symbols + (static_cast<uint32_t>(key[k] >> 32) & 31u);
      for (uint64_t open = __ballot(pending); open != 0; open = __ballot(pending)) {
         const uint32_t leader = static_cast<uint32_t>(__builtin_ctzll(open));
         const uint32_t leader_counter = __shfl(counter, leader);
         const uint64_t same = __ballot(pending && counter == leader_counter);
         if (lane == leader) {
            atomicAdd(&batch.counts[0][q][leader_counter], static_cast<uint32_t>(__popcll(same)));
         }
         if (counter == leader_counter) {
            pending = false;
         }
      }
   }
}

struct EscapeSliceArgs {
   const uint64_t* filters[SILO_GPU_MAX_SCAN_BATCH];
   uint32_t row_words;
   uint32_t n_slices;
   uint32_t n_ranges;
   uint32_t block_keys;
   const uint32_t* counters;
   double min_proportion[SILO_GPU_MAX_SCAN_BATCH];
   struct Range {
      const uint32_t* keys;
      const uint32_t* granule_base;
      const uint32_t* slice_first;
      const uint32_t* heaviest;
      const uint32_t* without;
      uint32_t positions;
      uint32_t pos_begin;
      uint32_t pos_end;
      uint32_t out_symbols;
      uint32_t key_from;
      uint32_t first_block;
      uint32_t blocks_per_slice;
      uint32_t* counts[SILO_GPU_MAX_SCAN_BATCH];
   } ranges[ESCAPE_MAX_RANGES];
};

static_assert(sizeof(EscapeSliceArgs) + sizeof(uint32_t) <= 4096, "k_scan_escapes_sliced takes its arguments by value: the kernel-argument segment holds 4 KiB");

__device__ __forceinline__ void ldsBarrier() {
   asm volatile("s_waitcnt lgkmcnt(0)\n\ts_barrier" ::: "memory");
}

constexpr uint32_t ESCAPE_GRANULES_PER_BLOCK = 64;
template <int FILTERS>
constexpr uint32_t escapeWindow() {
   return FILTERS >= 8 ? 896u : 12288u / FILTERS;
}
template <int FILTERS>
constexpr uint32_t escapeLdsBytes() {
   return (FILTERS * (ESCAPE_SLICE_WORDS32 + escapeWindow<FILTERS>()) + 3u * ESCAPE_GRANULES_PER_BLOCK + 4u + 64u) * static_cast<uint32_t>(sizeof(uint32_t));
}

template <int FILTERS>
__global__ __launch_bounds__(ESCAPE_SLICE_THREADS, FILTERS <= 4 ? 8 : 4) void k_scan_escapes_sliced(const EscapeSliceArgs args, uint32_t n_filters) {
   constexpr uint32_t WINDOW = escapeWindow<FILTERS>();
   static_assert(ESCAPE_GRANULE_KEYS == ESCAPE_SLICE_THREADS * 4u, "a granule is one 16-byte load per thread of the block");
   extern __shared__ uint32_t s_filter[];
   uint32_t* s_count = s_filter + FILTERS * ESCAPE_SLICE_WORDS32;
   uint32_t* s_base = s_count + FILTERS * WINDOW;
   uint32_t* s_end = s_base + ESCAPE_GRANULES_PER_BLOCK;
   uint32_t* s_live = s_end + ESCAPE_GRANULES_PER_BLOCK;
   uint32_t* s_nowhere = s_live + ESCAPE_GRANULES_PER_BLOCK + 4u;
   const uint32_t first_filter = blockIdx.z * FILTERS;
   uint32_t r = 0;
   while (r + 1u < args.n_ranges && blockIdx.x >= args.ranges[r + 1u].first_block) {
      ++r;
   }
   const EscapeSliceArgs::Range& range = args.ranges[r];
   const uint32_t slice = (blockIdx.x - range.first_block) / range.blocks_per_slice;
   const uint32_t share = (blockIdx.x - range.first_block) % range.blocks_per_slice;
   const uint32_t out_symbols = range.out_symbols;
   const uint32_t* first = range.slice_first + static_cast<size_t>(slice) * (range.positions + 1u);
   const uint32_t key_begin = first[range.key_from];
   const uint32_t key_end = first[range.pos_end];
   const uint32_t share_begin = key_begin / ESCAPE_GRANULE_KEYS * ESCAPE_GRANULE_KEYS + share * args.block_keys;
   if (share_begin >= key_end) {
      return;
   }
   const uint32_t share_end = min(share_begin + args.block_keys, key_end);
   const uint32_t range_first = range.pos_begin * out_symbols;
   const bool clamp = range.key_from < range.pos_begin;
   const uint32_t first_granule = share_begin / ESCAPE_GRANULE_KEYS;
   const uint32_t n_granules = (share_end - share_begin + ESCAPE_GRANULE_KEYS - 1u) / ESCAPE_GRANULE_KEYS;
   const auto loadGranule = [&](uint32_t granule) {
      const u32x4 v = __builtin_nontemporal_load(reinterpret_cast<const u32x4*>(range.keys + share_begin + granule * ESCAPE_GRANULE_KEYS + threadIdx.x * 4u));
      return make_uint4(v.x, v.y, v.z, v.w);
   };
   const bool prune = range.heaviest != nullptr;
   const auto listGranules = [&]() {
      if (threadIdx.x >= 64u) {
         return;
      }
      const bool in_share = threadIdx.x < n_granules;
      bool live = in_share;
      if (prune && in_share) {
         const uint32_t heaviest = range.heaviest[first_granule + threadIdx.x];
         const uint32_t without = range.without[first_granule + threadIdx.x];
         bool skip = true;
#pragma unroll
         for (int f = 0; f < FILTERS; ++f) {
            if (first_filter + f < n_filters) {
               skip = skip && granulePrunable(args.counters[(first_filter + f) * SPARSE_COUNTER_STRIDE + 2u], without, heaviest, args.min_proportion[first_filter + f]);
            }
         }
         live = !skip;
      }
      const uint64_t live_lanes = __ballot(live);
      if (live) {
         const uint32_t k = static_cast<uint32_t>(__popcll(live_lanes & ((uint64_t{1} << threadIdx.x) - 1u)));
         s_live[k] = threadIdx.x;
         s_base[k] = range.granule_base[first_granule + threadIdx.x];
         s_end[k] = threadIdx.x + 1u < n_granules ? range.granule_base[first_granule + threadIdx.x + 1u]
                                                  : range.granule_base[first_granule + threadIdx.x] + (range.keys[share_end - 1u] >> ESCAPE_SLICE_SHIFT) + 1u;
      }
      if (threadIdx.x == 0) {
         s_live[ESCAPE_GRANULES_PER_BLOCK] = static_cast<uint32_t>(__popcll(live_lanes));
      }
   };
   const auto liveGranule = [&](uint32_t k) { return static_cast<uint32_t>(__builtin_amdgcn_readfirstlane(static_cast<int>(s_live[k]))); };
   uint32_t n_live = n_granules;
   if (prune) {
      listGranules();
      __syncthreads();
      n_live = liveGranule(ESCAPE_GRANULES_PER_BLOCK);
      if (n_live == 0) {
         return;
      }
   }
   const auto loadKeys = [&](uint32_t k) {
      return loadGranule(liveGranule(min(k, n_live - 1u)));
   };
   uint64_t any_bit = 0;
   ulonglong2 filter_part[FILTERS][ESCAPE_SLICE_WORDS32 / 4u / ESCAPE_SLICE_THREADS];
#pragma unroll
   for (int f = 0; f < FILTERS; ++f) {
      const uint32_t first_word = slice * (ESCAPE_SLICE_WORDS32 / 2u);
      const bool present = first_filter + f < n_filters;
      const uint64_t* filter = args.filters[present ? first_filter + f : first_filter];
#pragma unroll
      for (uint32_t j = 0; j < ESCAPE_SLICE_WORDS32 / 4u / ESCAPE_SLICE_THREADS; ++j) {
         const uint32_t word = first_word + (j * ESCAPE_SLICE_THREADS + threadIdx.x) * 2u;
         filter_part[f][j] = present && word < args.row_words ? *reinterpret_cast<const ulonglong2*>(filter + word) : make_ulonglong2(0, 0);
      }
   }
   uint4 quad0 = prune ? loadKeys(0) : loadGranule(0);
   uint4 quad1 = prune ? loadKeys(1) : loadGranule(min(1u, n_granules - 1u));
   uint4 quad2 = prune ? loadKeys(2) : loadGranule(min(2u, n_granules - 1u));
   if (!prune) {
      listGranules();
   }
   constexpr bool BYTE_PER_ROW = FILTERS == 8;
   static_assert(ESCAPE_SLICE_WORDS32 / 4u / ESCAPE_SLICE_THREADS == 1u, "a thread holds one 16-byte part of a filter slice");
#pragma unroll
   for (int f = 0; f < FILTERS; ++f) {
      for (uint32_t j = threadIdx.x * 4u; j < WINDOW; j += ESCAPE_SLICE_THREADS * 4u) {
         *reinterpret_cast<uint4*>(s_count + f * WINDOW + j) = make_uint4(0, 0, 0, 0);
      }
      if constexpr (!BYTE_PER_ROW) {
         *reinterpret_cast<ulonglong2*>(s_filter + f * ESCAPE_SLICE_WORDS32 + threadIdx.x * 4u) = filter_part[f][0];
      }
      any_bit |= filter_part[f][0].x | filter_part[f][0].y;
   }
   if constexpr (BYTE_PER_ROW) {
#pragma unroll
      for (uint32_t quarter = 0; quarter < 4; ++quarter) {
         uint32_t bytes[8];
#pragma unroll
         for (uint32_t k = 0; k < 8; ++k) {
            bytes[k] = 0;
         }
#pragma unroll
         for (int f = 0; f < FILTERS; ++f) {
            const uint64_t half = quarter < 2 ? filter_part[f][0].x : filter_part[f][0].y;
            const uint32_t rows32 = static_cast<uint32_t>(half >> (32u * (quarter & 1u)));
#pragma unroll
            for (uint32_t k = 0; k < 8; ++k) {
               bytes[k] |= ((((rows32 >> (4u * k)) & 0xFu) * 0x00204081u) & 0x01010101u) << f;
            }
         }
         uint32_t* out = s_filter + threadIdx.x * 32u + quarter * 8u;
         *reinterpret_cast<uint4*>(out) = make_uint4(bytes[0], bytes[1], bytes[2], bytes[3]);
         *reinterpret_cast<uint4*>(out + 4) = make_uint4(bytes[4], bytes[5], bytes[6], bytes[7]);
      }
   }
   if (__syncthreads_or(any_bit != 0 ? 1 : 0) == 0) {
      return;
   }
   const uint32_t lane = __lane_id();
   uint32_t window_first = 0, window_used = 0, chunk_granules = 0, chunk_end = 0;
   const auto beginChunk = [&](uint32_t g) {
      const uint32_t first_counter = max(s_base[g], range_first);
      window_first = first_counter / out_symbols * out_symbols - range_first;
      uint32_t h = g + 1u;
      while (h < n_live && max(s_end[h], range_first) - range_first - window_first < WINDOW) {
         ++h;
      }
      chunk_granules = h;
      chunk_end = min(share_begin + (liveGranule(h - 1u) + 1u) * ESCAPE_GRANULE_KEYS, share_end);
      window_used = min(WINDOW, (max(s_end[h - 1u], range_first) / out_symbols + 1u) * out_symbols - range_first - window_first);
   };
   const auto flushChunk = [&]() {
      ldsBarrier();
#pragma unroll
      for (int f = 0; f < FILTERS; ++f) {
         uint32_t* __restrict__ counts = range.counts[first_filter + f < n_filters ? first_filter + f : first_filter] + window_first;
         for (uint32_t j = threadIdx.x; j < window_used; j += ESCAPE_SLICE_THREADS) {
            const uint32_t value = s_count[f * WINDOW + j];
            if (value != 0) {
               s_count[f * WINDOW + j] = 0;
               atomicAdd(&counts[j], value);
            }
         }
      }
      ldsBarrier();
   };
   const auto countGranule = [&](uint4& in_flight, uint32_t g) {
      if (g >= n_live) {
         return;
      }
      if (g == chunk_granules) {
         flushChunk();
         beginChunk(g);
      }
      const uint4 quad = in_flight;
      in_flight = loadKeys(g + 3u);
      const uint32_t granule_first = share_begin + liveGranule(g) * ESCAPE_GRANULE_KEYS;
      {
         const uint32_t granule_counter = s_base[g] - range_first - window_first;
         const uint32_t i = granule_first + threadIdx.x * 4u;
         const uint32_t keys4[4] = {quad.x, quad.y, quad.z, quad.w};
         uint32_t in_window[4];
         bool valid[4];
         if (granule_first >= key_begin && granule_first + ESCAPE_GRANULE_KEYS <= chunk_end) {
#pragma unroll
            for (uint32_t c = 0; c < 4; ++c) {
               valid[c] = keys4[c] != ESCAPE_KEY_INVALID;
            }
         } else {
#pragma unroll
            for (uint32_t c = 0; c < 4; ++c) {
               valid[c] = static_cast<bool>(static_cast<uint32_t>(keys4[c] != ESCAPE_KEY_INVALID) & static_cast<uint32_t>(i + c - key_begin < chunk_end - key_begin));
            }
         }
#pragma unroll
         for (uint32_t c = 0; c < 4; ++c) {
            in_window[c] = granule_counter + (keys4[c] >> ESCAPE_SLICE_SHIFT);
         }
         if (clamp && s_base[g] < range_first) {
#pragma unroll
            for (uint32_t c = 0; c < 4; ++c) {
               in_window[c] = static_cast<int32_t>(in_window[c]) < 0 ? in_window[c] & 1u : in_window[c];
            }
         }
         const uint32_t counter0 = in_window[0];
         const uint32_t previous = static_cast<uint32_t>(__builtin_amdgcn_update_dpp(0, static_cast<int>(counter0), 0x138 , 0xF, 0xF, false));
         const uint32_t following = static_cast<uint32_t>(__builtin_amdgcn_update_dpp(0, static_cast<int>(counter0), 0x130 , 0xF, 0xF, false));
         const bool head = lane == 0 || counter0 != previous;
         const bool tail = lane == 63 || counter0 != following;
         const uint64_t heads_at_or_below = __ballot(head) & (~uint64_t{0} >> (63u - lane));
         const uint32_t first_of_stretch = 63u - static_cast<uint32_t>(__builtin_clzll(heads_at_or_below));
         constexpr bool EVERY_KEY_IN_WINDOW = WINDOW >= ESCAPE_MAX_RELATIVE + 64u;
         [[maybe_unused]] uint32_t filters_with[4] = {0, 0, 0, 0};
         if constexpr (BYTE_PER_ROW) {
#pragma unroll
            for (uint32_t c = 0; c < 4; ++c) {
               filters_with[c] = reinterpret_cast<const uint8_t*>(s_filter)[keys4[c] & ESCAPE_ROW_MASK] & (valid[c] ? 0xFFu : 0u);
            }
         }
         if constexpr (BYTE_PER_ROW) {
            const auto add8 = [&](uint32_t counter, uint32_t value, int f) {
               const bool here = value != 0 && counter < WINDOW;
               if (__ballot(here) != 0) {
                  atomicAdd(here ? &s_count[f * WINDOW + counter] : &s_nowhere[lane], here ? value : 0u);
               }
               if (value != 0 && counter >= WINDOW) {
                  atomicAdd(&range.counts[first_filter + f < n_filters ? first_filter + f : first_filter][window_first + counter], value);
               }
            };
            uint32_t on_first = filters_with[0];
            uint32_t sums[4] = {0, 0, 0, 0};
            uint32_t elsewhere[4] = {0, 0, 0, 0};
#pragma unroll
            for (uint32_t c = 0; c < 4; ++c) {
               if (c != 0) {
                  const bool same = in_window[c] == counter0;
                  on_first = same ? filters_with[c] : 0u;
                  elsewhere[c] = same ? 0u : filters_with[c];
               }
#pragma unroll
               for (uint32_t k = 0; k < 4; ++k) {
                  sums[k] += ((on_first >> (2u * k)) & 1u) | (((on_first >> (2u * k + 1u)) & 1u) << 16);
               }
            }
#pragma unroll
            for (uint32_t k = 0; k < 4; ++k) {
               const uint32_t through = waveSumToLane63(sums[k]);
               const uint32_t before = through - sums[k];
               const uint32_t before_stretch = static_cast<uint32_t>(__builtin_amdgcn_ds_bpermute(static_cast<int>(first_of_stretch * 4u), static_cast<int>(before)));
               const uint32_t stretch = through - before_stretch;
               add8(counter0, tail ? stretch & 0xFFFFu : 0u, static_cast<int>(2u * k));
               add8(counter0, tail ? stretch >> 16 : 0u, static_cast<int>(2u * k + 1u));
            }
#pragma unroll
            for (uint32_t c = 1; c < 4; ++c) {
               if (__ballot(elsewhere[c] != 0) != 0) {
#pragma unroll
                  for (int f = 0; f < FILTERS; ++f) {
                     add8(in_window[c], (elsewhere[c] >> f) & 1u, f);
                  }
               }
            }
            return;
         }
#pragma unroll
         for (int f = 0; f < FILTERS; ++f) {
            uint32_t* __restrict__ window = s_count + f * WINDOW;
            [[maybe_unused]] uint32_t* __restrict__ table = range.counts[first_filter + f < n_filters ? first_filter + f : first_filter] + window_first;
            const auto add = [&](uint32_t counter, uint32_t value) {
               const bool here = EVERY_KEY_IN_WINDOW ? value != 0 : value != 0 && counter < WINDOW;
               atomicAdd(here ? &window[counter] : &s_nowhere[lane], here ? value : 0u);
               if constexpr (!EVERY_KEY_IN_WINDOW) {
                  if (value != 0 && counter >= WINDOW) {
                     atomicAdd(&table[counter], value);
                  }
               }
            };
            uint32_t n0 = 0;
            uint32_t elsewhere[4] = {0, 0, 0, 0};
#pragma unroll
            for (uint32_t c = 0; c < 4; ++c) {
               const uint32_t row = keys4[c] & ESCAPE_ROW_MASK;
               const uint32_t selected = (s_filter[f * ESCAPE_SLICE_WORDS32 + (row >> 5)] >> (row & 31u)) & (valid[c] ? 1u : 0u);
               if (c == 0) {
                  n0 = selected;
               } else {
                  const bool same = in_window[c] == counter0;
                  n0 += same ? selected : 0u;
                  elsewhere[c] = same ? 0u : selected;
               }
            }
            if (__ballot((elsewhere[1] | elsewhere[2] | elsewhere[3]) != 0) != 0) {
#pragma unroll
               for (uint32_t c = 1; c < 4; ++c) {
                  add(in_window[c], elsewhere[c]);
               }
            }
            const uint32_t through = waveSumToLane63(n0);
            const uint32_t before_stretch = static_cast<uint32_t>(__builtin_amdgcn_ds_bpermute(static_cast<int>(first_of_stretch * 4u), static_cast<int>(through - n0)));
            add(counter0, tail ? through - before_stretch : 0u);
         }
      }
   };
   beginChunk(0);
   for (uint32_t g = 0; g < n_live; g += 3u) {
      countGranule(quad0, g);
      countGranule(quad1, g + 1u);
      countGranule(quad2, g + 2u);
   }
   flushChunk();
}

__global__ __launch_bounds__(256) void k_scan_escapes_overflow(
   const uint64_t* __restrict__ keys, uint32_t n_keys, const ScanBatchArgs batch, uint32_t pos_begin, uint32_t pos_end
) {
   const uint32_t q = blockIdx.y;
   const uint32_t i = blockIdx.x * blockDim.x + threadIdx.x;
   if (i >= n_keys) {
      return;
   }
   const uint64_t key = keys[i];
   const uint32_t counter = static_cast<uint32_t>(key >> 32);
   const uint32_t sequence = static_cast<uint32_t>(key);
   if (counter >= pos_begin * batch.out_symbols && counter < pos_end * batch.out_symbols && ((batch.filters[q][sequence >> 6] >> (sequence & 63u)) & 1ull) != 0) {
      atomicAdd(&batch.counts[0][q][counter - pos_begin * batch.out_symbols], 1u);
   }
}

ScanBatchArgs keyBatch(const ScanRange& range, const uint64_t* const* filters, uint32_t q_count) {
   ScanBatchArgs batch{};
   batch.out_symbols = range.seqstore->dev.n_scan;
   copyFilters(batch.filters, filters, q_count);
   std::copy_n(range.counts, q_count, batch.counts[0]);
   return batch;
}

}

namespace silo_gpu_detail {

int scanEscapes(
   const std::vector<ScanRange>& ranges, const uint64_t* const* filters, uint32_t q_count, hipStream_t hip_stream, const std::vector<ScanRange>* gaps,
   const ScanPruning* pruning, const std::vector<ScanRange>* ends, bool only_ends
) {
   EscapeSliceArgs sliced{};
   copyFilters(sliced.filters, filters, q_count);
   const bool prune = gaps != nullptr && pruning != nullptr && pruning->keys;
   if (prune) {
      std::copy_n(pruning->min_proportion, q_count, sliced.min_proportion);
      sliced.counters = pruning->counters;
   }
   uint32_t n_sliced = 0;
   std::array<uint32_t, ESCAPE_MAX_RANGES> most_keys{};
   uint64_t total_keys = 0;
   bool end_entries = false;
   const auto launchSliced = [&]() -> int {
      if (n_sliced == 0) {
         return SILO_GPU_OK;
      }
      static std::once_flag lds_once;
      std::call_once(lds_once, [] {
         (void)hipFuncSetAttribute(reinterpret_cast<const void*>(k_scan_escapes_sliced<1>), hipFuncAttributeMaxDynamicSharedMemorySize, escapeLdsBytes<1>());
         (void)hipFuncSetAttribute(reinterpret_cast<const void*>(k_scan_escapes_sliced<2>), hipFuncAttributeMaxDynamicSharedMemorySize, escapeLdsBytes<2>());
         (void)hipFuncSetAttribute(reinterpret_cast<const void*>(k_scan_escapes_sliced<4>), hipFuncAttributeMaxDynamicSharedMemorySize, escapeLdsBytes<4>());
         (void)hipFuncSetAttribute(reinterpret_cast<const void*>(k_scan_escapes_sliced<8>), hipFuncAttributeMaxDynamicSharedMemorySize, escapeLdsBytes<8>());
      });
      const uint32_t per_block = q_count <= 1 ? 1 : (q_count <= 2 ? 2 : (q_count <= 4 ? 4 : 8));
      const uint32_t passes = (q_count + per_block - 1) / per_block;
      const uint64_t granules = (total_keys + ESCAPE_GRANULE_KEYS - 1) / ESCAPE_GRANULE_KEYS * passes;
      const uint32_t block_granules = static_cast<uint32_t>(std::min<uint64_t>(ESCAPE_GRANULES_PER_BLOCK, std::max<uint64_t>(1, granules / 1280)));
      const uint32_t block_keys = block_granules * ESCAPE_GRANULE_KEYS;
      sliced.block_keys = block_keys;
      sliced.n_ranges = n_sliced;
      uint32_t blocks = 0;
      for (uint32_t k = 0; k < n_sliced; ++k) {
         sliced.ranges[k].first_block = blocks;
         sliced.ranges[k].blocks_per_slice = std::max<uint32_t>(1, (most_keys[k] + block_keys - 1) / block_keys);
         blocks += sliced.ranges[k].blocks_per_slice * sliced.n_slices;
      }
      const dim3 grid(blocks, 1, passes);
      char name[64];
      bool bounds = false;
      for (uint32_t k = 0; k < n_sliced; ++k) {
         bounds = bounds || sliced.ranges[k].heaviest != nullptr;
      }
      std::snprintf(name, sizeof(name), "k_scan_escapes_sliced<%u>%s%s", per_block, bounds ? ", pruning" : "", end_entries ? ", ends" : "");
      ScanLaunchTiming* timing = startLaunchTiming(
         name, 0, total_keys * sizeof(uint32_t) * grid.z + static_cast<uint64_t>(grid.x) * q_count * ESCAPE_SLICE_WORDS32 * sizeof(uint32_t), q_count,
         grid.x * grid.z, hip_stream
      );
      switch (per_block) {
         case 1: k_scan_escapes_sliced<1><<<grid, ESCAPE_SLICE_THREADS, escapeLdsBytes<1>(), hip_stream>>>(sliced, q_count); break;
         case 2: k_scan_escapes_sliced<2><<<grid, ESCAPE_SLICE_THREADS, escapeLdsBytes<2>(), hip_stream>>>(sliced, q_count); break;
         case 4: k_scan_escapes_sliced<4><<<grid, ESCAPE_SLICE_THREADS, escapeLdsBytes<4>(), hip_stream>>>(sliced, q_count); break;
         default: k_scan_escapes_sliced<8><<<grid, ESCAPE_SLICE_THREADS, escapeLdsBytes<8>(), hip_stream>>>(sliced, q_count); break;
      }
      HIP_TRY(hipGetLastError());
      finishLaunchTiming(timing, hip_stream);
      n_sliced = 0;
      most_keys.fill(0);
      total_keys = 0;
      end_entries = false;
      return SILO_GPU_OK;
   };
   const auto addSliced = [&](const ScanRange& range, const SliceMajorKeys& stream, uint32_t out_symbols, uint32_t key_from, const uint32_t* heaviest = nullptr,
                              const uint32_t* without = nullptr) -> int {
      const uint32_t n_slices = stream.n_slices;
      if (n_sliced == ESCAPE_MAX_RANGES || (n_sliced != 0 && sliced.n_slices != n_slices)) {
         if (const int rc = launchSliced(); rc != SILO_GPU_OK) {
            return rc;
         }
      }
      sliced.row_words = range.seqstore->dev.row_words;
      sliced.n_slices = n_slices;
      EscapeSliceArgs::Range& entry = sliced.ranges[n_sliced];
      entry.keys = stream.d_keys.get();
      entry.granule_base = stream.d_granule_base.get();
      entry.slice_first = stream.d_slice_first.get();
      entry.heaviest = heaviest;
      entry.without = without;
      entry.positions = range.seqstore->dev.positions;
      entry.pos_begin = range.pos_begin;
      entry.pos_end = range.pos_end;
      entry.out_symbols = out_symbols;
      entry.key_from = key_from;
      std::copy_n(range.counts, q_count, entry.counts);
      const size_t stride = static_cast<size_t>(entry.positions) + 1;
      for (uint32_t slice = 0; slice < n_slices; ++slice) {
         const uint32_t n = stream.slice_first[slice * stride + range.pos_end] - stream.slice_first[slice * stride + key_from];
         total_keys += n;
         most_keys[n_sliced] = std::max(most_keys[n_sliced], n + ESCAPE_GRANULE_KEYS - 1u);
      }
      ++n_sliced;
      return SILO_GPU_OK;
   };
   const auto addGaps = [&](size_t r) -> int {
      const SeqStoreHost::Layout& layout = ranges[r].seqstore->layout;
      if (gaps == nullptr || (*gaps)[r].seqstore == nullptr || layout.gaps.d_keys.get() == nullptr) {
         return SILO_GPU_OK;
      }
      return addSliced((*gaps)[r], layout.gaps, 2, 0);
   };
   const auto addEnds = [&](size_t r) -> int {
      const SeqStoreHost::Layout& layout = ranges[r].seqstore->layout;
      if (ends == nullptr || (*ends)[r].seqstore == nullptr || layout.ends.d_keys.get() == nullptr) {
         return SILO_GPU_OK;
      }
      if (const int rc = addSliced((*ends)[r], layout.ends, 2, 0); rc != SILO_GPU_OK) {
         return rc;
      }
      end_entries = true;
      if (layout.residual.d_keys.get() == nullptr) {
         return SILO_GPU_OK;
      }
      const int rc = addSliced(ranges[r], layout.residual, ranges[r].seqstore->dev.n_scan, ranges[r].pos_begin);
      end_entries = true;
      return rc;
   };
   for (size_t r = 0; r < ranges.size(); ++r) {
      const ScanRange& range = ranges[r];
      const SeqStoreHost::Layout& layout = range.seqstore->layout;
      if (const int rc = addEnds(r); rc != SILO_GPU_OK) {
         return rc;
      }
      if (only_ends) {
         continue;
      }
      const uint32_t begin = layout.built && layout.d_escapes.get() != nullptr ? layout.escape_first[range.pos_begin] : 0;
      const uint32_t count = layout.built && layout.d_escapes.get() != nullptr ? layout.escape_first[range.pos_end] - begin : 0;
      if (count == 0) {
         if (const int rc = addGaps(r); rc != SILO_GPU_OK) {
            return rc;
         }
         continue;
      }
      const SliceMajorKeys& keys = layout.escapes_sliced;
      if (keys.d_keys.get() != nullptr && g_tune_side_stream.load() != 3) {
         if (keys.n_overflow != 0) {
            k_scan_escapes_overflow<<<dim3((keys.n_overflow + 255) / 256, q_count), 256, 0, hip_stream>>>(
               keys.d_overflow.get(), keys.n_overflow, keyBatch(range, filters, q_count), range.pos_begin, range.pos_end
            );
            HIP_TRY(hipGetLastError());
         }
         const bool bounds = prune && layout.d_granule_heaviest.get() != nullptr && layout.d_granule_without.get() != nullptr;
         if (const int rc = addSliced(
                range, keys, range.seqstore->dev.n_scan, range.pos_begin, bounds ? layout.d_granule_heaviest.get() : nullptr,
                bounds ? layout.d_granule_without.get() : nullptr
             );
             rc != SILO_GPU_OK) {
            return rc;
         }
         if (const int rc = addGaps(r); rc != SILO_GPU_OK) {
            return rc;
         }
         continue;
      }
      if (const int rc = addGaps(r); rc != SILO_GPU_OK) {
         return rc;
      }
      const uint32_t keys_per_block = 256 * ESCAPE_KEYS_PER_THREAD;
      k_scan_escapes<<<dim3((count + keys_per_block - 1) / keys_per_block, q_count), 256, 0, hip_stream>>>(
         layout.d_escapes.get() + begin, count, keyBatch(range, filters, q_count), range.pos_begin
      );
      HIP_TRY(hipGetLastError());
   }
   return launchSliced();
}

}
```

lapis-silo_amd/csrc/store_internal.h:

```cpp
#pragma once
#include <hip/hip_runtime.h>

#include <stdint.h>
#include <string.h>

#include <atomic>
#include <memory>
#include <mutex>
#include <string>
#include <vector>

#include "../../include/silo_gpu.h"
#include "bitprog.h"
#include "internal.h"
#include "layout_choice.h"

extern std::atomic<int> g_tune_rows_per_block;
extern std::atomic<int> g_tune_scan_variant;
extern std::atomic<int> g_tune_eval_leaf_batch;
extern std::atomic<int> g_tune_compact_index;
extern std::atomic<int> g_tune_gap_events;
extern std::atomic<int> g_tune_prune_keys;
extern std::atomic<int> g_tune_end_runs;
extern std::atomic<int> g_tune_fused_select;
extern std::atomic<int> g_tune_side_stream;
extern std::atomic<int> g_tune_scan_timing;
extern std::atomic<int> g_tune_missing_runs;
extern std::atomic<int> g_tune_key_cost;
extern std::atomic<int> g_tune_launch_cost;
extern std::atomic<int> g_tune_sparse_divisor;

struct silo_gpu_row_slot {
   uint32_t capacity = 0;
   uint32_t epoch = 0;
   silo_gpu_detail::DeviceArray<uint32_t> d_cursor_and_ticket;
   void* host = nullptr;
   void* host_dev = nullptr;
};

namespace silo_gpu_detail {

inline int fail(int code, const std::string& message) {
   return silo_gpu_internal_fail(code, message);
}

#define HIP_TRY(expr) SILO_HIP_TRY(expr)

inline int failHip(const std::string& what, hipError_t status) {
   (void)hipGetLastError();
   return fail(status == hipErrorOutOfMemory ? SILO_GPU_ERR_OUT_OF_MEMORY : SILO_GPU_ERR_HIP, what + ": " + hipGetErrorString(status));
}

constexpr uint32_t ROW_ALIGN_WORDS = 32;

inline void fillCharTable(uint32_t alphabet, uint8_t table[256]) {
   memset(table, SILO_GPU_SYMBOL_NONE, 256);
   if (alphabet == SILO_GPU_ALPHABET_NUCLEOTIDE) {
      const char* symbols = "-ACGTRYSWKMBDHVN";
      for (int i = 0; i < 16; ++i) {
         table[static_cast<uint8_t>(symbols[i])] = static_cast<uint8_t>(i);
      }
      table[static_cast<uint8_t>('.')] = 0;
      table[static_cast<uint8_t>('U')] = 4;
   } else {
      const char* symbols = "-ACDEFGHIKLMNPQRSTVWYBZ*X";
      for (int i = 0; i < 25; ++i) {
         table[static_cast<uint8_t>(symbols[i])] = static_cast<uint8_t>(i);
      }
   }
}

inline uint32_t alphabetSize(uint32_t alphabet) {
   return alphabet == SILO_GPU_ALPHABET_NUCLEOTIDE ? SILO_GPU_NUC_SYMBOLS : SILO_GPU_AA_SYMBOLS;
}
inline uint32_t missingSymbol(uint32_t alphabet) {
   return alphabet == SILO_GPU_ALPHABET_NUCLEOTIDE ? 15u : 24u;
}


enum : uint8_t { PLANE_SPARSE = 0, PLANE_SCAN = 1, PLANE_EXTRA = 2, PLANE_RUNS = 3 };
enum : uint32_t { BUILD_PLANES = 0, BUILD_COUNT = 1, BUILD_ENCODE = 2 };


using silo_gpu_layout::LAYOUT_IDENTITY;
using silo_gpu_layout::LAYOUT_ONE_HOT;
using silo_gpu_layout::LAYOUT_IMPLICIT;
using silo_gpu_layout::LAYOUT_ROWS_MASK;
using silo_gpu_layout::IMPLICIT_SLOT;
using silo_gpu_layout::CODE_MAP_STRIDE;

struct SeqStoreDev {
   uint64_t* scan;
   uint64_t* extra;
   const uint64_t* missing_run_keys;
   const uint32_t* missing_run_ends;
   uint32_t n_missing_runs;
   uint32_t build_mode;
   uint32_t* enc_counts;
   const uint8_t* enc_code_map;
   const uint32_t* enc_row_of;
   uint64_t* enc_planes;
   const uint32_t* enc_first;
   uint32_t* enc_cursor;
   uint64_t* enc_escapes;
   uint32_t runs_at_build;
   unsigned long long* enc_run_count;
   uint64_t* enc_run_keys;
   uint32_t* enc_run_ends;
   unsigned long long enc_run_capacity;
   const uint64_t* planes;
   const uint32_t* row_of;
   const uint8_t* code_map;
   const uint64_t* escapes;
   const uint32_t* escape_first;
   uint32_t positions;
   uint32_t n_symbols;
   uint32_t n_scan;
   uint32_t n_bits;
   uint32_t n_extra;
   uint32_t row_words;
   uint32_t missing_symbol;
   uint8_t kind[SILO_GPU_MAX_SYMBOLS];
   uint8_t index[SILO_GPU_MAX_SYMBOLS];
};

__host__ __device__ inline uint64_t* planePtr(const SeqStoreDev& s, uint32_t position, uint32_t symbol) {
   const uint8_t kind = s.kind[symbol];
   if (kind == PLANE_EXTRA) {
      return s.extra + (static_cast<size_t>(s.index[symbol]) * s.positions + position) * s.row_words;
   }
   return nullptr;
}

struct PositionLayout {
   const uint64_t* rows;
   uint32_t bits;
   bool identity;
   bool one_hot;
   bool implicit;
   const uint8_t* map;
};
__device__ __forceinline__ PositionLayout layoutOf(const SeqStoreDev& s, uint32_t position) {
   if (s.code_map == nullptr) {
      return {s.planes + static_cast<size_t>(position) * s.n_bits * s.row_words, s.n_bits, true, false, false, nullptr};
   }
   const uint8_t* map = s.code_map + static_cast<size_t>(position) * CODE_MAP_STRIDE;
   return {s.planes + static_cast<size_t>(s.row_of[position]) * s.row_words, static_cast<uint32_t>(map[0] & LAYOUT_ROWS_MASK), (map[0] & LAYOUT_IDENTITY) != 0,
           (map[0] & LAYOUT_ONE_HOT) != 0, (map[0] & LAYOUT_IMPLICIT) != 0, map};
}

constexpr uint32_t CODE_ESCAPED = 0xFFFFFFFFu;
constexpr uint32_t CODE_IMPLICIT = 0xFFFFFFFEu;
__device__ __forceinline__ uint32_t codeOfSymbol(const PositionLayout& layout, uint32_t scan_index) {
   if (layout.identity) {
      return scan_index + 1u;
   }
   if (layout.implicit && layout.map[IMPLICIT_SLOT] == scan_index) {
      return CODE_IMPLICIT;
   }
   const uint32_t n_codes = layout.one_hot ? layout.bits + 1u : (1u << layout.bits);
   for (uint32_t code = 1; code < n_codes; ++code) {
      if (layout.map[code] == scan_index) {
         return code;
      }
   }
   return CODE_ESCAPED;
}

__device__ __forceinline__ uint64_t decodeCodeWord(const PositionLayout& layout, uint32_t row_words, uint32_t code, uint32_t word) {
   if (layout.one_hot) {
      return layout.rows[static_cast<size_t>(code - 1u) * row_words + word];
   }
   uint64_t match = ~0ull;
   for (uint32_t bit = 0; bit < layout.bits; ++bit) {
      const uint64_t plane_word = layout.rows[static_cast<size_t>(bit) * row_words + word];
      match &= ((code >> bit) & 1u) != 0 ? plane_word : ~plane_word;
   }
   return match;
}

__device__ __forceinline__ uint32_t codeOfRow(const PositionLayout& layout, uint32_t row_words, uint32_t word, uint32_t bit) {
   uint32_t code = 0;
   for (uint32_t plane = 0; plane < layout.bits; ++plane) {
      const uint32_t set = static_cast<uint32_t>((layout.rows[static_cast<size_t>(plane) * row_words + word] >> bit) & 1u);
      code = layout.one_hot ? (set != 0 ? plane + 1u : code) : (code | (set << plane));
   }
   return code;
}

struct SliceMajorKeys {
   DeviceArray<uint32_t> d_keys;
   DeviceArray<uint32_t> d_granule_base;
   DeviceArray<uint64_t> d_overflow;
   uint32_t n_overflow = 0;
   uint64_t packed_keys = 0;
   uint32_t n_slices = 0;
   DeviceArray<uint32_t> d_slice_first;
   std::vector<uint32_t> slice_first;
};

struct SeqStoreHost {
   SeqStoreDev dev{};
   uint32_t alphabet = 0;
   std::vector<uint8_t> reference;
   DeviceArray<uint8_t> d_reference;
   DeviceArray<uint64_t> d_sparse;
   uint32_t sparse_capacity = 0;
   DeviceArray<uint32_t> d_sparse_count;
   std::vector<uint64_t> sparse_sorted;
   bool finalized = false;
   uint64_t rows_filled = 0;
   std::vector<uint8_t> imported_positions;
   DeviceArray<uint32_t> d_totals;
   bool totals_ready = false;
   DeviceArray<uint64_t> d_row_hashes;
   bool row_hashes_ready = false;
   DeviceArray<uint32_t> d_row_cell_counts;
   bool row_cell_counts_ready = false;
   DeviceArray<uint64_t> d_scan;
   DeviceArray<uint64_t> d_extra;
   DeviceArray<uint64_t> d_missing_run_keys;
   DeviceArray<uint32_t> d_missing_run_ends;
   struct LayoutWork;
   std::shared_ptr<LayoutWork> work;
   DeviceArray<unsigned long long> d_run_count;
   struct Run {
      uint32_t begin;
      uint32_t end;
      uint8_t bits;
      bool identity;
      bool one_hot;
   };
   struct Layout {
      bool built = false;
      DeviceArray<uint64_t> planes;
      DeviceArray<uint32_t> d_row_of;
      DeviceArray<uint32_t> d_row_target;
      DeviceArray<uint8_t> d_code_map;
      DeviceArray<uint64_t> d_escapes;
      DeviceArray<uint32_t> d_escape_first;
      SliceMajorKeys escapes_sliced;
      uint32_t slice_shift = 0;
      std::vector<uint32_t> row_of;
      std::vector<uint8_t> code_map;
      std::vector<uint32_t> escape_first;
      std::vector<uint32_t> escape_first_symbol;
      std::vector<Run> runs;
      uint64_t device_bytes = 0;
      bool has_implicit = false;
      DeviceArray<uint32_t> d_run_slice_first;
      uint32_t n_run_slices = 0;
      bool gap_stream = false;
      SliceMajorKeys gaps;
      DeviceArray<uint32_t> d_granule_heaviest;
      DeviceArray<uint32_t> d_granule_without;
      std::vector<uint32_t> granule_heaviest;
      std::vector<uint32_t> granule_without;
      DeviceArray<uint32_t> d_row_heaviest;
      DeviceArray<uint32_t> d_row_without;
      std::vector<uint32_t> row_heaviest;
      std::vector<uint32_t> row_without;
      DeviceArray<uint32_t> d_end_lead;
      DeviceArray<uint32_t> d_end_trail;
      SliceMajorKeys ends;
      uint64_t end_events = 0;
      SliceMajorKeys residual;
      uint64_t residual_keys = 0;
      DeviceArray<uint8_t> d_row_covered;
      DeviceArray<uint8_t> d_position_covered;
      std::vector<uint8_t> row_covered;
      std::vector<uint8_t> position_covered;
      uint64_t covered_rows = 0;
      uint32_t end_symbol = 0;
   } layout;
};

struct SeqStoreHost::LayoutWork {
   std::vector<uint8_t> code_map;
   std::vector<uint32_t> row_of, row_target, escape_first, escape_first_symbol;
   std::vector<Run> runs;
   uint64_t total_rows = 0, total_escapes = 0;
   size_t plane_bytes = 0, escape_bytes = 0;
   bool has_implicit = false;
   DeviceArray<uint8_t> d_code_map;
   DeviceArray<uint32_t> d_cursor;
   DeviceArray<uint32_t> d_first;
   DeviceArray<uint32_t> d_row_of;
   DeviceArray<uint32_t> d_row_target;
   DeviceArray<uint32_t> d_escape_first;
   DeviceArray<uint64_t> d_planes;
   DeviceArray<uint64_t> d_escapes;
};

}

struct silo_gpu_store {
   int device = 0;
   uint32_t sequence_count = 0;
   uint32_t row_words = 0;
   uint64_t device_bytes = 0;
   std::vector<silo_gpu_detail::SeqStoreHost> seqstores;
   silo_gpu_detail::DeviceArray<uint64_t> d_ones;
   silo_gpu_detail::DeviceArray<uint16_t> d_lineage;
   uint32_t n_lineages = 0;
   silo_gpu_detail::DeviceArray<uint32_t> d_error_flag;
   silo_gpu_detail::DeviceArray<uint8_t> d_stage;
   size_t stage_capacity = 0;
   silo_gpu_detail::DeviceArray<uint8_t> d_stage_null;
   size_t stage_null_capacity = 0;
   silo_gpu_detail::DeviceArray<uint64_t> d_import_row;
   silo_gpu_detail::DeviceArray<uint64_t> d_import_union;
   silo_gpu_store_options options{SILO_GPU_OPTION_DEFAULT, SILO_GPU_OPTION_DEFAULT, SILO_GPU_OPTION_DEFAULT, SILO_GPU_OPTION_DEFAULT};
   silo_gpu_detail::DeviceArray<uint8_t> d_char_table[2];
   silo_gpu_detail::DeviceArray<char> d_symbol_chars[2];
   std::mutex mutex;
};

namespace silo_gpu_detail {

inline int layoutOption(const silo_gpu_store* store) {
   return store->options.layout != SILO_GPU_OPTION_DEFAULT ? store->options.layout : g_tune_compact_index.load();
}
inline int missingRunsOption(const silo_gpu_store* store) {
   return store->options.missing_runs != SILO_GPU_OPTION_DEFAULT ? store->options.missing_runs : g_tune_missing_runs.load();
}
inline int keyCostOption(const silo_gpu_store* store) {
   return store->options.key_cost != SILO_GPU_OPTION_DEFAULT ? store->options.key_cost : g_tune_key_cost.load();
// ... 95 lines not shown
```

lapis-silo_amd/silo_amd/binding.py:

```python
import ctypes
import os

import numpy as np

from . import alphabet

_LIB_DIR = os.path.join(os.path.dirname(os.path.dirname(os.path.abspath(__file__))), "lib")
_LIB_PATH = os.path.join(_LIB_DIR, "libsilo_gpu.so")

c_u8p = ctypes.POINTER(ctypes.c_uint8)
c_u16p = ctypes.POINTER(ctypes.c_uint16)
c_u32p = ctypes.POINTER(ctypes.c_uint32)
c_u64p = ctypes.POINTER(ctypes.c_uint64)


class SiloGpuError(RuntimeError):
    def __init__(self, code, message):
        super().__init__(f"silo_gpu error {code}: {message}")
        self.code = code


class SeqStoreDesc(ctypes.Structure):
    _fields_ = [
        ("alphabet", ctypes.c_uint32),
        ("positions", ctypes.c_uint32),
        ("reference", c_u8p),
        ("n_scan_symbols", ctypes.c_uint32),
        ("scan_symbols", c_u8p),
        ("n_extra_symbols", ctypes.c_uint32),
        ("extra_symbols", c_u8p),
    ]


class StoreDesc(ctypes.Structure):
    _fields_ = [
        ("device", ctypes.c_int32),
        ("sequence_count", ctypes.c_uint32),
        ("n_seqstores", ctypes.c_uint32),
        ("seqstores", ctypes.POINTER(SeqStoreDesc)),
    ]


class SynthDesc(ctypes.Structure):
    _fields_ = [
        ("seed", ctypes.c_uint64),
        ("n_lineages", ctypes.c_uint32),
        ("lineage_of_sequence", c_u16p),
        ("lead_gap", c_u32p),
        ("trail_gap", c_u32p),
        ("missing_start", c_u32p),
        ("missing_len", c_u32p),
        ("lineage_symbol", c_u8p),
        ("private_threshold", ctypes.c_uint32),
        ("ambiguous_threshold", ctypes.c_uint32),
        ("position_offset", ctypes.c_uint32),
        ("total_positions", ctypes.c_uint32),
    ]


class RoaringPayload(ctypes.Structure):
    _fields_ = [("symbol", ctypes.c_uint32), ("bytes", ctypes.c_char_p), ("n_bytes", ctypes.c_size_t)]


class ScanTiming(ctypes.Structure):
    _fields_ = [("kernel", ctypes.c_char * 64), ("plane_rows", ctypes.c_uint64), ("bytes", ctypes.c_uint64), ("filters", ctypes.c_uint32),
                ("blocks", ctypes.c_uint32), ("ms", ctypes.c_float)]


def scan_timings(capacity=64):
    lib = load_library()
    out = (ScanTiming * capacity)()
    n = ctypes.c_uint32()
    _check(lib.silo_gpu_scan_timings(out, capacity, ctypes.byref(n)))
    return [dict(kernel=out[k].kernel.decode(), plane_rows=int(out[k].plane_rows), bytes=int(out[k].bytes), filters=int(out[k].filters), blocks=int(out[k].blocks),
                 ms=float(out[k].ms))
            for k in range(min(capacity, n.value))]


class BitProg(ctypes.Structure):
    _fields_ = [
        ("n_instructions", ctypes.c_uint32),
        ("code", c_u32p),
        ("n_leaves", ctypes.c_uint32),
        ("leaves", ctypes.POINTER(ctypes.c_void_p)),
        ("n_slots", ctypes.c_uint32),
    ]


EXPORTED_SYMBOLS = [
    "silo_gpu_store_create", "silo_gpu_store_destroy", "silo_gpu_store_set_options", "silo_gpu_store_sequence_count",
    "silo_gpu_store_row_words", "silo_gpu_store_device_bytes", "silo_gpu_store_append_sequences",
    "silo_gpu_store_finalize", "silo_gpu_store_generate_synthetic", "silo_gpu_bitset_alloc",
    "silo_gpu_bitset_upload", "silo_gpu_bitset_download", "silo_gpu_bitset_from_lineages", "silo_gpu_upload_u32",
    "silo_gpu_bitset_from_value_ids", "silo_gpu_free",
    "silo_gpu_malloc", "silo_gpu_memcpy_d2h", "silo_gpu_memcpy_h2d", "silo_gpu_stream_synchronize", "silo_gpu_stream_create", "silo_gpu_set_device", "silo_gpu_stream_destroy", "silo_gpu_store_plane",
    "silo_gpu_store_sparse_plane", "silo_gpu_filter_eval", "silo_gpu_filter_eval_batch", "silo_gpu_popcount", "silo_gpu_mutations_scan", "silo_gpu_mutations_scan_batch", "silo_gpu_mutations_scan_ranges", "silo_gpu_mutations_grouped", "silo_gpu_store_scan_planes", "silo_gpu_store_scan_escapes", "silo_gpu_store_scan_overflow_keys", "silo_gpu_store_scan_rows", "silo_gpu_store_scan_runs", "silo_gpu_row_slot_create", "silo_gpu_row_slot_destroy", "silo_gpu_mutations_select_to_slot", "silo_gpu_row_slot_wait", "silo_gpu_store_scan_sparse_keys", "silo_gpu_store_finalize_seqstore", "silo_gpu_store_build_pass", "silo_gpu_store_build_mode", "silo_gpu_store_memory_info", "silo_gpu_store_import_position", "silo_gpu_store_import_missing_rows",
    "silo_gpu_memset_async", "silo_gpu_event_create", "silo_gpu_event_record", "silo_gpu_event_elapsed_ms",
    "silo_gpu_event_destroy", "silo_gpu_event_synchronize", "silo_gpu_host_alloc", "silo_gpu_host_free", "silo_gpu_memcpy_d2h_async", "silo_gpu_mutations_select", "silo_gpu_upload_bytes", "silo_gpu_upload_column", "silo_gpu_bitset_from_compare", "silo_gpu_group_count", "silo_gpu_group_count_hashed", "silo_gpu_reconstruct_sequences", "silo_gpu_bitset_from_pairs", "silo_gpu_count_pairs", "silo_gpu_count_slot_create", "silo_gpu_count_slot_destroy", "silo_gpu_filter_eval_count", "silo_gpu_count_slot_wait", "silo_gpu_tune", "silo_gpu_last_scan_kernel", "silo_gpu_scan_timings", "silo_gpu_stream_read_probe", "silo_gpu_last_error",
    "silo_gpu_comm_unique_id", "silo_gpu_comm_create", "silo_gpu_comm_destroy", "silo_gpu_comm_rank", "silo_gpu_comm_world",
    "silo_gpu_allreduce_counts", "silo_gpu_broadcast_bytes",
    "silo_gpu_mutations_scan_select",
    "silo_gpu_mutations_scan_ranges_min_proportion", "silo_gpu_store_scan_prunable_granules", "silo_gpu_store_scan_prunable_rows",
    "silo_gpu_store_scan_covered_rows", "silo_gpu_store_scan_end_events", "silo_gpu_store_scan_residual_keys",
    "silo_gpu_filters_grouped", "silo_gpu_filters_cross",
    "silo_gpu_distance_pack", "silo_gpu_distance_pairs", "silo_gpu_distance_within", "silo_gpu_adjacency_components",
    "silo_gpu_distance_weights", "silo_gpu_spanning_forest", "silo_gpu_distance_listed_pairs",
    "silo_gpu_distance_cross", "silo_gpu_nearest_columns",
    "silo_gpu_consensus_call",
    "silo_gpu_query_distances", "silo_gpu_nearest_rows", "silo_gpu_bitset_from_distances",
    "silo_gpu_position_symbols", "silo_gpu_haplotype_ids",
    "silo_gpu_mutations_compare",
    "silo_gpu_sequence_differences",
    "silo_gpu_sample_key", "silo_gpu_sample_groups", "silo_gpu_sample_begin", "silo_gpu_sample_count", "silo_gpu_sample_advance",
    "silo_gpu_sample_select",
    "silo_gpu_row_hash_term", "silo_gpu_row_hashes", "silo_gpu_store_row_hashes", "silo_gpu_distinct_begin", "silo_gpu_distinct_insert",
    "silo_gpu_distinct_select",
    "silo_gpu_distinct_count", "silo_gpu_distinct_classes", "silo_gpu_smallest_keys",
    "silo_gpu_row_cell_counts", "silo_gpu_store_row_cell_counts", "silo_gpu_bitset_from_cell_counts", "silo_gpu_cell_count_histogram",
]

_lib = None


def load_library():
    global _lib
    if _lib is not None:
        return _lib
    if not os.path.exists(_LIB_PATH):
        raise ImportError(
            f"{_LIB_PATH} is missing: run `python -c 'import __graft_entry__ as g; g.build()'` "
            "(hipcc --offload-arch=gfx950). The product path has no CPU fallback."
        )
    lib = ctypes.CDLL(_LIB_PATH)
    vp = ctypes.c_void_p
    lib.silo_gpu_store_create.argtypes = [ctypes.POINTER(StoreDesc), ctypes.POINTER(vp)]
    lib.silo_gpu_store_destroy.argtypes = [vp]
    lib.silo_gpu_store_destroy.restype = None
    lib.silo_gpu_store_sequence_count.argtypes = [vp]
    lib.silo_gpu_store_sequence_count.restype = ctypes.c_uint32
    lib.silo_gpu_store_row_words.argtypes = [vp]
    lib.silo_gpu_store_row_words.restype = ctypes.c_uint32
    lib.silo_gpu_store_device_bytes.argtypes = [vp]
    lib.silo_gpu_store_device_bytes.restype = ctypes.c_uint64
    lib.silo_gpu_store_append_sequences.argtypes = [vp, ctypes.c_uint32, ctypes.c_uint32, ctypes.c_uint32, vp, vp]
    lib.silo_gpu_store_finalize.argtypes = [vp]
    lib.silo_gpu_store_generate_synthetic.argtypes = [vp, ctypes.c_uint32, ctypes.POINTER(SynthDesc)]
    lib.silo_gpu_bitset_alloc.argtypes = [vp, ctypes.POINTER(vp)]
    lib.silo_gpu_bitset_upload.argtypes = [vp, vp, vp, ctypes.c_size_t, vp]
    lib.silo_gpu_bitset_download.argtypes = [vp, vp, vp, ctypes.c_size_t, vp]
    lib.silo_gpu_bitset_from_lineages.argtypes = [vp, vp, vp, ctypes.c_uint32, vp]
    lib.silo_gpu_free.argtypes = [vp]
    lib.silo_gpu_free.restype = None
    lib.silo_gpu_malloc.argtypes = [ctypes.c_size_t, ctypes.POINTER(vp)]
    lib.silo_gpu_memcpy_d2h.argtypes = [vp, vp, ctypes.c_size_t, vp]
    lib.silo_gpu_memcpy_h2d.argtypes = [vp, vp, ctypes.c_size_t, vp]
    lib.silo_gpu_upload_u32.argtypes = [vp, ctypes.c_size_t, ctypes.POINTER(vp)]
    lib.silo_gpu_bitset_from_value_ids.argtypes = [vp, vp, vp, vp, ctypes.c_uint32, vp]
    lib.silo_gpu_stream_synchronize.argtypes = [vp]
    lib.silo_gpu_stream_create.argtypes = [ctypes.POINTER(vp)]
    lib.silo_gpu_stream_destroy.argtypes = [vp]
    lib.silo_gpu_stream_destroy.restype = None
    lib.silo_gpu_store_plane.argtypes = [vp, ctypes.c_uint32, ctypes.c_uint32, ctypes.c_uint32]
    lib.silo_gpu_store_plane.restype = vp
    lib.silo_gpu_store_sparse_plane.argtypes = [vp, ctypes.c_uint32, ctypes.c_uint32, ctypes.c_uint32, vp, vp]
    lib.silo_gpu_filter_eval.argtypes = [vp, ctypes.POINTER(BitProg), vp, vp, vp]
    lib.silo_gpu_popcount.argtypes = [vp, vp, vp, vp]
    lib.silo_gpu_mutations_scan.argtypes = [vp, ctypes.c_uint32, vp, ctypes.c_uint32, ctypes.c_uint32, vp, vp]
    lib.silo_gpu_mutations_scan_batch.argtypes = [vp, ctypes.c_uint32, ctypes.POINTER(vp), ctypes.c_uint32, ctypes.c_uint32, ctypes.c_uint32, ctypes.POINTER(vp), vp]
    lib.silo_gpu_store_scan_planes.argtypes = [vp, ctypes.c_uint32]
    lib.silo_gpu_store_scan_planes.restype = ctypes.c_uint32
    lib.silo_gpu_store_scan_escapes.argtypes = [vp, ctypes.c_uint32]
    lib.silo_gpu_store_scan_escapes.restype = ctypes.c_uint64
    lib.silo_gpu_store_scan_overflow_keys.argtypes = [vp, ctypes.c_uint32]
    lib.silo_gpu_store_scan_overflow_keys.restype = ctypes.c_uint64
    lib.silo_gpu_mutations_scan_ranges.argtypes = [vp, ctypes.POINTER(ctypes.c_uint32), ctypes.c_uint32, ctypes.POINTER(vp), ctypes.c_uint32, ctypes.POINTER(vp), vp]
    lib.silo_gpu_mutations_scan_ranges_min_proportion.argtypes = [vp, ctypes.POINTER(ctypes.c_uint32), ctypes.c_uint32, ctypes.POINTER(vp), ctypes.c_uint32,
                                                                  ctypes.POINTER(ctypes.c_double), ctypes.POINTER(vp), vp]
    lib.silo_gpu_mutations_scan_select.argtypes = [vp, ctypes.POINTER(ctypes.c_uint32), ctypes.c_uint32, ctypes.POINTER(vp), ctypes.c_uint32,
                                                   ctypes.POINTER(ctypes.c_double), ctypes.POINTER(vp), ctypes.POINTER(SelectSink), vp]
    lib.silo_gpu_store_scan_prunable_granules.argtypes = [vp, ctypes.c_uint32, ctypes.c_uint32, ctypes.c_double, ctypes.POINTER(ctypes.c_uint64),
                                                          ctypes.POINTER(ctypes.c_uint64)]
    lib.silo_gpu_store_scan_prunable_rows.argtypes = lib.silo_gpu_store_scan_prunable_granules.argtypes
    for name in ("silo_gpu_store_scan_covered_rows", "silo_gpu_store_scan_end_events", "silo_gpu_store_scan_residual_keys"):
        getattr(lib, name).argtypes = [vp, ctypes.c_uint32]
        getattr(lib, name).restype = ctypes.c_uint64
    lib.silo_gpu_mutations_grouped.argtypes = [vp, ctypes.c_uint32, vp, vp, vp, ctypes.c_uint32, vp, vp, ctypes.c_uint32, vp, vp, vp]
    lib.silo_gpu_filters_grouped.argtypes = [vp, vp, vp, vp, ctypes.c_uint32, ctypes.POINTER(vp), ctypes.c_uint32, vp, vp, vp]
    lib.silo_gpu_filters_cross.argtypes = [vp, vp, ctypes.POINTER(vp), vp, ctypes.c_uint32, ctypes.POINTER(vp), vp, ctypes.c_uint32, vp, vp,
                                           ctypes.c_uint32, ctypes.c_uint32, vp]
    lib.silo_gpu_distance_pack.argtypes = [ctypes.c_int, vp, ctypes.c_uint32, ctypes.c_uint32, vp, vp]
    lib.silo_gpu_distance_pairs.argtypes = [ctypes.c_int, vp, ctypes.c_uint32, ctypes.c_uint32, vp, vp]
    lib.silo_gpu_distance_within.argtypes = [ctypes.c_int, vp, ctypes.c_uint32, ctypes.c_uint32, ctypes.c_uint32, ctypes.c_uint32, vp, vp]
    lib.silo_gpu_adjacency_components.argtypes = [vp, ctypes.c_uint32, vp, vp, vp]
    lib.silo_gpu_distance_weights.argtypes = [ctypes.c_int, vp, ctypes.c_uint32, ctypes.c_uint32, ctypes.c_uint32, ctypes.c_uint32, vp, vp]
    lib.silo_gpu_spanning_forest.argtypes = [vp, ctypes.c_uint32, vp, vp, vp]
    lib.silo_gpu_distance_listed_pairs.argtypes = [ctypes.c_int, vp, ctypes.c_uint32, ctypes.c_uint32, vp, vp, ctypes.c_uint32, vp, vp]
    lib.silo_gpu_distance_cross.argtypes = [ctypes.c_int, vp, ctypes.c_uint32, vp, ctypes.c_uint32, ctypes.c_uint32, vp, ctypes.c_uint32,
                                            ctypes.c_uint32, vp, vp]
    lib.silo_gpu_nearest_columns.argtypes = [vp, ctypes.c_uint32, ctypes.c_uint32, ctypes.c_uint32, vp, vp, vp]
    lib.silo_gpu_consensus_call.argtypes = [ctypes.c_int, vp, ctypes.c_uint32, ctypes.c_uint32, vp, ctypes.c_double, ctypes.c_uint32, vp, vp, vp]
    lib.silo_gpu_query_distances.argtypes = [vp, ctypes.c_uint32, vp, vp, vp, vp]
    lib.silo_gpu_nearest_rows.argtypes = [vp, vp, ctypes.c_uint32, ctypes.c_uint32, ctypes.c_uint32, ctypes.c_uint32, vp, vp, vp, vp]
    lib.silo_gpu_bitset_from_distances.argtypes = [vp, ctypes.c_uint32, ctypes.c_uint32, ctypes.c_uint32, ctypes.c_uint32, vp, vp]
    lib.silo_gpu_position_symbols.argtypes = [vp, ctypes.c_uint32, vp, ctypes.c_uint32, vp, vp, vp]
    lib.silo_gpu_haplotype_ids.argtypes = [vp, ctypes.c_uint32, ctypes.c_uint32, ctypes.c_uint32, ctypes.c_uint32, ctypes.c_uint32, vp,
                                           ctypes.POINTER(vp), vp, vp]
    lib.silo_gpu_mutations_compare.argtypes = [ctypes.c_int, vp, ctypes.c_uint32, ctypes.c_uint32, vp, ctypes.c_double, ctypes.c_double,
                                               ctypes.c_uint32, vp, vp]
    lib.silo_gpu_sequence_differences.argtypes = [ctypes.c_int, vp, ctypes.c_uint32, ctypes.c_uint32, vp, ctypes.c_uint32, vp, vp, vp, vp, vp]
    lib.silo_gpu_sample_key.argtypes = [ctypes.c_uint64, ctypes.c_uint32]
    lib.silo_gpu_sample_key.restype = ctypes.c_uint32
    lib.silo_gpu_sample_groups.argtypes = [vp, vp, vp, ctypes.c_uint32, ctypes.c_uint32, ctypes.c_uint32, vp, vp]
    lib.silo_gpu_sample_begin.argtypes = [vp, ctypes.c_uint32, ctypes.c_uint32, ctypes.c_uint64, vp]
    lib.silo_gpu_sample_count.argtypes = [vp, vp, vp, ctypes.c_uint32, ctypes.c_uint32, ctypes.c_uint32, ctypes.c_uint32, vp]
    lib.silo_gpu_sample_advance.argtypes = [vp, ctypes.c_uint32, vp]
    lib.silo_gpu_sample_select.argtypes = [vp, vp, vp, ctypes.c_uint32, ctypes.c_uint32, ctypes.c_uint32, vp, vp]
    lib.silo_gpu_row_hash_term.argtypes = [ctypes.c_uint32, ctypes.c_uint32, ctypes.c_uint32]
    lib.silo_gpu_row_hash_term.restype = ctypes.c_uint64
    lib.silo_gpu_row_hashes.argtypes = [vp, ctypes.c_uint32, vp, vp, vp]
    lib.silo_gpu_store_row_hashes.argtypes = [vp, ctypes.c_uint32, ctypes.POINTER(vp), vp]
    lib.silo_gpu_distinct_begin.argtypes = [vp, ctypes.c_uint32, vp]
    lib.silo_gpu_distinct_insert.argtypes = [vp, ctypes.c_uint32, vp, ctypes.c_uint32, ctypes.c_uint32, vp, vp]
    lib.silo_gpu_distinct_select.argtypes = [vp, ctypes.c_uint32, vp, ctypes.c_uint32, ctypes.c_uint32, vp, vp, vp]
    lib.silo_gpu_distinct_count.argtypes = [vp, ctypes.c_uint32, vp, vp, ctypes.c_uint32, ctypes.c_uint32, vp, vp]
    lib.silo_gpu_distinct_classes.argtypes = [vp, ctypes.c_uint32, vp, vp, ctypes.c_uint32, ctypes.c_uint32, vp, ctypes.c_uint32, vp, ctypes.c_uint32,
                                              vp, vp]
    lib.silo_gpu_smallest_keys.argtypes = [vp, vp, ctypes.c_uint32, ctypes.c_uint32, vp, vp, vp, vp]
    lib.silo_gpu_row_cell_counts.argtypes = [vp, ctypes.c_uint32, vp, vp, vp]
    lib.silo_gpu_store_row_cell_counts.argtypes = [vp, ctypes.c_uint32, ctypes.POINTER(vp), vp]
    lib.silo_gpu_bitset_from_cell_counts.argtypes = [vp, ctypes.c_uint32, ctypes.c_uint32, ctypes.c_uint32, ctypes.c_uint32, ctypes.c_uint32, vp, vp]
    lib.silo_gpu_cell_count_histogram.argtypes = [vp, ctypes.c_uint32, ctypes.c_uint32, vp, ctypes.c_uint32, ctypes.c_uint32, ctypes.c_uint32, vp, vp]
    lib.silo_gpu_memset_async.argtypes = [vp, ctypes.c_int, ctypes.c_size_t, vp]
    lib.silo_gpu_upload_column.argtypes = [vp, ctypes.c_size_t, ctypes.c_int, ctypes.POINTER(vp)]
    lib.silo_gpu_bitset_from_compare.argtypes = [vp, vp, vp, ctypes.c_int, ctypes.c_int, vp, vp]
    lib.silo_gpu_group_count.argtypes = [vp, vp, ctypes.POINTER(vp), ctypes.POINTER(ctypes.c_uint32), ctypes.c_uint32, vp, vp]
    lib.silo_gpu_mutations_select.argtypes = [vp, vp, ctypes.c_uint32, ctypes.c_uint32, ctypes.c_double, ctypes.c_uint32, vp, vp]
    lib.silo_gpu_upload_bytes.argtypes = [vp, ctypes.c_size_t, ctypes.POINTER(vp)]
    lib.silo_gpu_count_slot_create.argtypes = [ctypes.POINTER(vp)]
    lib.silo_gpu_count_slot_destroy.argtypes = [vp]
    lib.silo_gpu_count_slot_destroy.restype = None
    lib.silo_gpu_filter_eval_count.argtypes = [vp, ctypes.POINTER(BitProg), vp, vp, vp]
    lib.silo_gpu_count_slot_wait.argtypes = [vp, c_u64p, vp]
    lib.silo_gpu_row_slot_create.argtypes = [ctypes.c_uint32, ctypes.POINTER(vp)]
    lib.silo_gpu_row_slot_destroy.argtypes = [vp]
    lib.silo_gpu_row_slot_destroy.restype = None
    lib.silo_gpu_mutations_select_to_slot.argtypes = [vp, vp, ctypes.c_uint32, ctypes.c_uint32, ctypes.c_double, vp, vp]
    lib.silo_gpu_row_slot_wait.argtypes = [vp, ctypes.POINTER(vp), c_u32p, vp]
    lib.silo_gpu_bitset_from_pairs.argtypes = [vp, vp, vp, vp, ctypes.c_uint32, vp, ctypes.c_uint32, vp]
    lib.silo_gpu_count_pairs.argtypes = [vp, vp, vp, vp, ctypes.c_uint32, vp, vp]
    lib.silo_gpu_group_count_hashed.argtypes = [vp, vp, ctypes.POINTER(vp), ctypes.POINTER(ctypes.c_uint32), ctypes.c_uint32, ctypes.c_uint32,
                                                ctypes.POINTER(vp), ctypes.POINTER(vp), ctypes.POINTER(ctypes.c_uint32), vp]
    lib.silo_gpu_reconstruct_sequences.argtypes = [vp, ctypes.c_uint32, vp, ctypes.c_uint32, vp, vp]
    lib.silo_gpu_event_create.argtypes = [ctypes.POINTER(vp)]
    lib.silo_gpu_event_record.argtypes = [vp, vp]
    lib.silo_gpu_event_elapsed_ms.argtypes = [vp, vp, ctypes.POINTER(ctypes.c_float)]
    lib.silo_gpu_event_destroy.argtypes = [vp]
    lib.silo_gpu_event_destroy.restype = None
    lib.silo_gpu_tune.argtypes = [ctypes.c_int, ctypes.c_int]
    lib.silo_gpu_last_scan_kernel.restype = ctypes.c_char_p
    lib.silo_gpu_store_build_pass.argtypes = [vp, ctypes.c_uint32, ctypes.c_int]
    lib.silo_gpu_store_build_pass.restype = ctypes.c_int
    lib.silo_gpu_store_build_mode.argtypes = [vp, ctypes.c_uint32]
    lib.silo_gpu_store_build_mode.restype = ctypes.c_int
    lib.silo_gpu_scan_timings.argtypes = [ctypes.POINTER(ScanTiming), ctypes.c_uint32, ctypes.POINTER(ctypes.c_uint32)]
    lib.silo_gpu_scan_timings.restype = ctypes.c_int
    lib.silo_gpu_last_error.restype = ctypes.c_char_p
    lib.silo_gpu_stream_read_probe.argtypes = [ctypes.c_uint64, ctypes.c_uint32, ctypes.POINTER(ctypes.c_float)]
    lib.silo_gpu_stream_read_probe.restype = ctypes.c_int
    lib.silo_gpu_store_scan_rows.argtypes = [vp, ctypes.c_uint32, ctypes.c_uint32, ctypes.c_uint32]
    lib.silo_gpu_store_scan_rows.restype = ctypes.c_uint64
    for name in ("silo_gpu_store_scan_runs", "silo_gpu_store_scan_sparse_keys"):
        getattr(lib, name).argtypes = [vp, ctypes.c_uint32]
        getattr(lib, name).restype = ctypes.c_uint64
    lib.silo_gpu_store_finalize_seqstore.argtypes = [vp, ctypes.c_uint32]
    lib.silo_gpu_store_import_position.argtypes = [vp, ctypes.c_uint32, ctypes.c_uint32, ctypes.POINTER(RoaringPayload), ctypes.c_uint32, ctypes.c_uint32,
                                                   ctypes.c_uint32]
    lib.silo_gpu_store_import_missing_rows.argtypes = [vp, ctypes.c_uint32, ctypes.c_uint32, ctypes.c_uint32, ctypes.POINTER(RoaringPayload)]
    lib.silo_gpu_filter_eval_batch.argtypes = [vp, ctypes.POINTER(BitProg), ctypes.c_uint32, ctypes.POINTER(vp), c_u64p, vp]
    lib.silo_gpu_comm_unique_id.argtypes = [vp]
    lib.silo_gpu_comm_create.argtypes = [vp, ctypes.c_uint32, ctypes.c_uint32, ctypes.c_int, ctypes.POINTER(vp)]
    lib.silo_gpu_comm_destroy.argtypes = [vp]
    lib.silo_gpu_comm_destroy.restype = None
    lib.silo_gpu_comm_rank.argtypes = [vp]
    lib.silo_gpu_comm_rank.restype = ctypes.c_uint32
    lib.silo_gpu_comm_world.argtypes = [vp]
    lib.silo_gpu_comm_world.restype = ctypes.c_uint32
    lib.silo_gpu_allreduce_counts.argtypes = [vp, vp, ctypes.c_size_t, vp]
    lib.silo_gpu_broadcast_bytes.argtypes = [vp, vp, ctypes.c_size_t, ctypes.c_uint32, vp]
    _lib = lib
    return lib


COMM_ID_BYTES = 128


def comm_unique_id():
    buffer = (ctypes.c_uint8 * COMM_ID_BYTES)()
    _check(load_library().silo_gpu_comm_unique_id(buffer))
    return bytes(buffer)


class Comm:

    def __init__(self, unique_id, rank, world, device=0):
        self.lib = load_library()
        if len(unique_id) != COMM_ID_BYTES:
            raise ValueError("a communicator id has %d bytes" % COMM_ID_BYTES)
        handle = ctypes.c_void_p()
        _check(self.lib.silo_gpu_comm_create((ctypes.c_uint8 * COMM_ID_BYTES).from_buffer_copy(unique_id), rank, world, device, ctypes.byref(handle)))
        self.handle = handle
        self.rank, self.world = rank, world

    def all_reduce_counts(self, device_ptr, n, stream=None):
        _check(self.lib.silo_gpu_allreduce_counts(self.handle, device_ptr, n, stream))

    def broadcast_bytes(self, device_ptr, nbytes, root, stream=None):
        _check(self.lib.silo_gpu_broadcast_bytes(self.handle, device_ptr, nbytes, root, stream))

    def close(self):
        if getattr(self, "handle", None):
            self.lib.silo_gpu_comm_destroy(self.handle)
            self.handle = None


def _check(rc):
    if rc != 0:
        raise SiloGpuError(rc, load_library().silo_gpu_last_error().decode())


def _ptr(array):
    return array.ctypes.data_as(ctypes.c_void_p)


class GpuEvent:

    def __init__(self):
        self.lib = load_library()
        self.handle = ctypes.c_void_p()
        _check(self.lib.silo_gpu_event_create(ctypes.byref(self.handle)))

    def record(self, stream=None):
        _check(self.lib.silo_gpu_event_record(self.handle, stream))

    def elapsed_ms(self, stop):
        ms = ctypes.c_float()
        _check(self.lib.silo_gpu_event_elapsed_ms(self.handle, stop.handle, ctypes.byref(ms)))
        return ms.value

    def __del__(self):
        if getattr(self, "handle", None):
            self.lib.silo_gpu_event_destroy(self.handle)
            self.handle = None


class GpuStream:

    def __init__(self):
        self.lib = load_library()
        self.handle = ctypes.c_void_p()
        _check(self.lib.silo_gpu_stream_create(ctypes.byref(self.handle)))

    def synchronize(self):
        _check(self.lib.silo_gpu_stream_synchronize(self.handle))

    def close(self):
        if getattr(self, "handle", None):
            self.lib.silo_gpu_stream_destroy(self.handle)
            self.handle = None


class CountSlot:

    def __init__(self):
        self.lib = load_library()
        self.handle = ctypes.c_void_p()
        _check(self.lib.silo_gpu_count_slot_create(ctypes.byref(self.handle)))

    def wait(self, stream=None):
        count = ctypes.c_uint64()
        _check(self.lib.silo_gpu_count_slot_wait(self.handle, ctypes.byref(count), stream))
        return int(count.value)

    def close(self):
        if getattr(self, "handle", None):
            self.lib.silo_gpu_count_slot_destroy(self.handle)
            self.handle = None


class SelectSink(ctypes.Structure):
    _fields_ = [("table_dev", ctypes.c_void_p), ("total_positions", ctypes.c_uint32), ("n_symbols", ctypes.c_uint32),
                ("reference_index_dev", ctypes.c_void_p), ("slot", ctypes.c_void_p)]


class RowSlot:

    def __init__(self, capacity):
        self.lib = load_library()
        self.capacity = int(capacity)
        self.handle = ctypes.c_void_p()
        _check(self.lib.silo_gpu_row_slot_create(self.capacity, ctypes.byref(self.handle)))

    def wait(self, stream=None):
        rows, n = ctypes.c_void_p(), ctypes.c_uint32()
        _check(self.lib.silo_gpu_row_slot_wait(self.handle, ctypes.byref(rows), ctypes.byref(n), stream))
        delivered = min(n.value, self.capacity)
        table = np.frombuffer(ctypes.string_at(rows.value, 16 * delivered), dtype=np.uint32).reshape(-1, 4)
        return int(n.value), table

    def close(self):
        if getattr(self, "handle", None):
            self.lib.silo_gpu_row_slot_destroy(self.handle)
            self.handle = None


(OP_LOAD, OP_ZERO, OP_ONES, OP_NOT, OP_AND, OP_OR, OP_ANDNOT, OP_CNT_ADD, OP_CNT_GE, OP_CNT_EQ, OP_MOV,
 OP_OR_N, OP_AND_N, OP_CNT_ADD_N, OP_CNT_ADD_NOT_N) = range(15)


COUNT_SHARDS = 64
LEAF_OPERAND = 32


def encode(op, dst=0, a=0, b=0, imm=0):
    return [op | (dst << 8) | (a << 16) | (b << 24), imm]


class PreparedPrograms:

    def __init__(self, programs, out_bitsets=None):
        self.n = len(programs)
        self.array = (BitProg * max(1, self.n))()
        self._keep = []
        for k, (code, leaves, n_slots) in enumerate(programs):
            code = np.ascontiguousarray(code, dtype=np.uint32)
            leaf_array = (ctypes.c_void_p * max(1, len(leaves)))(*[(l.value if isinstance(l, ctypes.c_void_p) else l) for l in leaves])
            self._keep += [code, leaf_array]
            self.array[k] = BitProg(len(code) // 2, code.ctypes.data_as(c_u32p), len(leaves), leaf_array, n_slots)
        self.outs = None
        if out_bitsets is not None:
            self.outs = (ctypes.c_void_p * max(1, self.n))(*[(o.value if isinstance(o, ctypes.c_void_p) else o) for o in out_bitsets])
        self.counts = np.zeros(max(1, self.n), dtype=np.uint64)

    def launch(self, store_handle, stream=None):
        _check(load_library().silo_gpu_filter_eval_batch(store_handle, self.array, self.n, self.outs, self.counts.ctypes.data_as(c_u64p), stream))
        return [int(c) for c in self.counts[:self.n]]


SYMBOL_NONE = 0xFF


def import_position(store_handle, seqstore_id, position, payloads, flipped=None, deleted=None):
    items = sorted(payloads.items())
    array = (RoaringPayload * max(1, len(items)))(*[RoaringPayload(symbol, data, len(data)) for symbol, data in items])
    _check(load_library().silo_gpu_store_import_position(
        store_handle, seqstore_id, position, array, len(items), SYMBOL_NONE if flipped is None else flipped, SYMBOL_NONE if deleted is None else deleted))


def import_missing_rows(store_handle, seqstore_id, first_sequence, payloads):
    array = (RoaringPayload * max(1, len(payloads)))(*[RoaringPayload(0, data, len(data)) for data in payloads])
    _check(load_library().silo_gpu_store_import_missing_rows(store_handle, seqstore_id, first_sequence, len(payloads), array))


def filter_eval_batch(store_handle, programs, out_bitsets=None, stream=None):
    return PreparedPrograms(programs, out_bitsets).launch(store_handle, stream)


MAX_DATE_RANGES = 1024
MAX_GROUPED_MUTATIONS = 4096
MAX_GROUPED_FILTERS = 2048
MAX_CROSS_FILTERS = 1024
CROSS_TILE = 8
CROSS_CHUNK_WORDS = 1024
_OWN_SCRATCH = object()


def grouped_scratch_bytes(row_words, n_ranges, n_mutations):
    return row_words * 128 + n_mutations * 32 + n_ranges * 16 + n_ranges * 4 * (1 + 3 * n_mutations) + 1024


def filters_grouped_scratch_bytes(row_words, n_ranges, n_filters):
    return row_words * 128 + n_filters * 8 + n_ranges * 16 + 1024


def filters_cross_scratch_bytes(n_rows, n_cols):
    return (n_rows + n_cols) * 16 + 1024


MAX_DISTANCE_ROWS = 2048
DISTANCE_TILE = 16
DISTANCE_CHUNK_WORDS = 32


def _abi_alphabet(name_or_id):
    return alphabet.ALPHABETS[name_or_id].abi_id if isinstance(name_or_id, str) else int(name_or_id)


def distance_planes(alphabet_id):
    return 6 if _abi_alphabet(alphabet_id) == 1 else 4


def distance_words(positions):
    return (positions + 63) // 64


def device_malloc(nbytes, fill=None, stream=None):
    lib = load_library()
    ptr = ctypes.c_void_p()
    _check(lib.silo_gpu_malloc(max(1, nbytes), ctypes.byref(ptr)))
    if fill is not None and nbytes:
        _check(lib.silo_gpu_memset_async(ptr, fill, nbytes, stream))
    return ptr


def device_free(ptr):
    load_library().silo_gpu_free(ptr)


def device_read(ptr, dtype, count, stream=None):
    out = np.empty(count, dtype=dtype)
    if count:
        _check(load_library().silo_gpu_memcpy_d2h(_ptr(out), ptr, out.nbytes, stream))
    return out


def distance_pack(alphabet_id, chars, fill=None, stream=None):
    lib = load_library()
    chars = np.ascontiguousarray(chars, dtype=np.uint8)
    n_rows, positions = chars.shape
    abi = _abi_alphabet(alphabet_id)
    planes = device_malloc(n_rows * distance_planes(abi) * distance_words(positions) * 8, fill, stream)
    chars_dev = device_malloc(chars.size)
    try:
        if chars.size:
            _check(lib.silo_gpu_memcpy_h2d(chars_dev, _ptr(chars), chars.size, stream))
        _check(lib.silo_gpu_distance_pack(abi, chars_dev, n_rows, positions, planes, stream))
        _check(lib.silo_gpu_stream_synchronize(stream))
    except Exception:
        device_free(planes)
        raise
    finally:
        device_free(chars_dev)
    return planes


def distance_pairs(alphabet_id, planes_ptr, n_rows, positions, fill=None, stream=None):
    lib = load_library()
    cells = n_rows * n_rows * 2
    out = device_malloc(cells * 4, fill, stream)
    try:
        _check(lib.silo_gpu_distance_pairs(_abi_alphabet(alphabet_id), planes_ptr, n_rows, positions, out, stream))
        _check(lib.silo_gpu_stream_synchronize(stream))
        return device_read(out, np.uint32, cells, stream).reshape(n_rows, n_rows, 2)
    finally:
        device_free(out)


MAX_CLUSTER_ROWS = 8192
WITHIN_TILE_ROWS = 16
WITHIN_TILE_COLS = 64
WITHIN_CHUNK_WORDS = 16
COMPONENTS_THREADS = 1024

# ... 1227 lines not shown
```

Baseline: 1854000 billion positions*sequences/s.

## Add persistent escape-scan blocks and order never-pruned ranges first

The escape scan now plans its work as items: ranges that can never be pruned come first, and block size is derived from their keys per resident block. An optional tune knob launches a grid-strided persistent kernel. That kernel walks items, reuses the loaded filter slice and zeroed counters when the slice repeats, and skips slices whose filter has no rows. This is meant to balance load and cut launch and reload overhead, at the cost of extra kernel variants, an occupancy query and more complex control flow.

```diff
diff --git a/include/silo_gpu.h b/include/silo_gpu.h
--- a/include/silo_gpu.h
+++ b/include/silo_gpu.h
@@ -508,6 +508,7 @@
        SILO_GPU_TUNE_PRUNE_KEYS = 11 ,
        SILO_GPU_TUNE_END_RUNS = 12 ,
        SILO_GPU_TUNE_FUSED_SELECT = 13 ,
+       SILO_GPU_TUNE_ESCAPE_BLOCKS = 14 ,
        SILO_GPU_TUNE_SCAN_SPARSE_DIVISOR = 3  };
 int silo_gpu_tune(int knob, int value);
 
@@ -528,6 +529,7 @@
 int silo_gpu_broadcast_bytes(silo_gpu_comm* comm, void* bytes_dev, size_t n_bytes, uint32_t root, void* stream);
 
 const char* silo_gpu_last_scan_kernel(void);
+uint32_t silo_gpu_last_escape_items(void);
 
 typedef struct silo_gpu_scan_timing {
    char kernel[64];
diff --git a/lapis-silo_amd/csrc/escape_item_plan.h b/lapis-silo_amd/csrc/escape_item_plan.h
--- /dev/null
+++ b/lapis-silo_amd/csrc/escape_item_plan.h
@@ -0,0 +1,96 @@
+#pragma once
+#include <stddef.h>
+#include <stdint.h>
+
+#include <algorithm>
+
+namespace silo_gpu_detail {
+
+constexpr uint32_t ESCAPE_PLAN_MAX_ENTRIES = 16;
+constexpr uint32_t ESCAPE_PLAN_GRANULE_KEYS = 4096;
+constexpr uint32_t ESCAPE_PLAN_GRANULES_PER_ITEM = 64;
+constexpr uint32_t ESCAPE_PLAN_MAX_ITEMS = 1u << 30;
+
+struct EscapeEntryShape {
+   uint32_t most_keys;
+   uint64_t keys;
+   bool prunable;
+};
+
+struct EscapeItemPlan {
+   bool ok;
+   uint32_t block_keys;
+   uint32_t n_items;
+   uint32_t grid;
+   bool never_pruned_first;
+   uint32_t order[ESCAPE_PLAN_MAX_ENTRIES];
+   uint32_t first_item[ESCAPE_PLAN_MAX_ENTRIES];
+   uint32_t items_per_slice[ESCAPE_PLAN_MAX_ENTRIES];
+};
+
+struct EscapeItem {
+   uint32_t entry;
+   uint32_t slice;
+   uint32_t share;
+};
+inline EscapeItem escapeItemOf(const EscapeItemPlan& plan, uint32_t n_entries, uint32_t item) {
+   uint32_t k = 0;
+   while (k + 1u < n_entries && item >= plan.first_item[k + 1u]) {
+      ++k;
+   }
+   const uint32_t within = item - plan.first_item[k];
+   return EscapeItem{k, within / plan.items_per_slice[k], within % plan.items_per_slice[k]};
+}
+
+inline uint64_t escapeItemsPerSlice(const EscapeEntryShape& entry, uint32_t block_keys) {
+   return std::max<uint64_t>(1, (static_cast<uint64_t>(entry.most_keys) + block_keys - 1) / block_keys);
+}
+
+inline EscapeItemPlan planEscapeItems(const EscapeEntryShape* entries, uint32_t n_entries, uint32_t n_slices, uint32_t passes, uint32_t places, int knob) {
+   EscapeItemPlan plan{};
+   if (entries == nullptr || n_entries == 0 || n_entries > ESCAPE_PLAN_MAX_ENTRIES || n_slices == 0 || passes == 0) {
+      return plan;
+   }
+   const uint32_t resident = knob > 0 ? static_cast<uint32_t>(knob) : std::max<uint32_t>(1, places / passes);
+   bool prunable = false;
+   uint64_t keys = 0, never_pruned_keys = 0;
+   for (uint32_t k = 0; k < n_entries; ++k) {
+      prunable = prunable || entries[k].prunable;
+      keys += entries[k].keys;
+      never_pruned_keys += entries[k].prunable ? 0 : entries[k].keys;
+   }
+   const auto granulesOf = [](uint64_t n) { return (n + ESCAPE_PLAN_GRANULE_KEYS - 1) / ESCAPE_PLAN_GRANULE_KEYS; };
+   const uint64_t never_pruned_per_place = granulesOf(never_pruned_keys) / resident;
+   const bool never_pruned_first = prunable && never_pruned_per_place >= 2;
+   const uint64_t granules = never_pruned_first ? std::max(never_pruned_per_place, granulesOf(keys - never_pruned_keys) * passes / 1280)
+                                                : granulesOf(keys) * passes / 1280;
+   const uint32_t block_granules = static_cast<uint32_t>(std::min<uint64_t>(ESCAPE_PLAN_GRANULES_PER_ITEM, std::max<uint64_t>(1, granules)));
+   plan.block_keys = block_granules * ESCAPE_PLAN_GRANULE_KEYS;
+   uint64_t items = 0;
+   for (uint32_t k = 0; k < n_entries; ++k) {
+      items += escapeItemsPerSlice(entries[k], plan.block_keys) * n_slices;
+   }
+   if (items > ESCAPE_PLAN_MAX_ITEMS) {
+      return plan;
+   }
+   uint32_t n = 0, first = 0;
+   for (const bool pruned : {false, true}) {
+      for (uint32_t k = 0; k < n_entries; ++k) {
+         if (never_pruned_first ? entries[k].prunable != pruned : pruned) {
+            continue;
+         }
+         plan.order[n] = k;
+         plan.first_item[n] = first;
+         plan.items_per_slice[n] = static_cast<uint32_t>(escapeItemsPerSlice(entries[k], plan.block_keys));
+         first += plan.items_per_slice[n] * n_slices;
+         ++n;
+      }
+   }
+   plan.n_items = first;
+   plan.grid = knob == 0 ? plan.n_items : std::min(plan.n_items, resident);
+   plan.never_pruned_first = never_pruned_first;
+   plan.ok = true;
+   return plan;
+}
+
+}
diff --git a/lapis-silo_amd/csrc/scan_internal.h b/lapis-silo_amd/csrc/scan_internal.h
--- a/lapis-silo_amd/csrc/scan_internal.h
+++ b/lapis-silo_amd/csrc/scan_internal.h
@@ -149,6 +149,7 @@
 int scanPiecesGather(const std::vector<ScanPiece> (&pieces)[N_SCAN_LAYOUTS], const SeqStoreDev& any_store, const uint64_t* const* filters, uint32_t q_count,
    const uint32_t* sparse_sectors, uint32_t sparse_capacity, const uint32_t* sector_index, uint32_t stride, hipStream_t hip_stream);
 
+extern thread_local uint32_t g_last_escape_items;
 int scanEscapes(const std::vector<ScanRange>& ranges, const uint64_t* const* filters, uint32_t q_count, hipStream_t hip_stream, const std::vector<ScanRange>* gaps, const ScanPruning* pruning,
    const std::vector<ScanRange>* ends = nullptr, bool only_ends = false);
 
diff --git a/lapis-silo_amd/csrc/silo_gpu_runtime.hip b/lapis-silo_amd/csrc/silo_gpu_runtime.hip
--- a/lapis-silo_amd/csrc/silo_gpu_runtime.hip
+++ b/lapis-silo_amd/csrc/silo_gpu_runtime.hip
@@ -29,6 +29,7 @@
 std::atomic<int> g_tune_prune_keys{0};
 std::atomic<int> g_tune_end_runs{0};
 std::atomic<int> g_tune_fused_select{0};
+std::atomic<int> g_tune_escape_blocks{0};
 
 namespace {
 thread_local std::string g_last_error;
@@ -89,6 +90,9 @@
    }
    if (knob == SILO_GPU_TUNE_FUSED_SELECT) {
       return g_tune_fused_select.exchange(value);
+   }
+   if (knob == SILO_GPU_TUNE_ESCAPE_BLOCKS) {
+      return g_tune_escape_blocks.exchange(value);
    }
    return -1;
 }
diff --git a/lapis-silo_amd/csrc/silo_gpu_scan.hip b/lapis-silo_amd/csrc/silo_gpu_scan.hip
--- a/lapis-silo_amd/csrc/silo_gpu_scan.hip
+++ b/lapis-silo_amd/csrc/silo_gpu_scan.hip
@@ -510,6 +510,10 @@
    return g_last_scan_kernel;
 }
 
+uint32_t silo_gpu_last_escape_items(void) {
+   return g_last_escape_items;
+}
+
 int silo_gpu_mutations_scan_ranges(
    const silo_gpu_store* store, const silo_gpu_scan_range* ranges, uint32_t n_ranges, const uint64_t* const* filters_dev, uint32_t n_filters,
    uint32_t* const* counts_out_dev, void* stream
diff --git a/lapis-silo_amd/csrc/silo_gpu_scan_keys.hip b/lapis-silo_amd/csrc/silo_gpu_scan_keys.hip
--- a/lapis-silo_amd/csrc/silo_gpu_scan_keys.hip
+++ b/lapis-silo_amd/csrc/silo_gpu_scan_keys.hip
@@ -5,11 +5,13 @@
 
 #include <algorithm>
 #include <array>
+#include <atomic>
 #include <mutex>
 #include <string>
 #include <type_traits>
 #include <vector>
 
+#include "escape_item_plan.h"
 #include "scan_internal.h"
 
 using namespace silo_gpu_detail;
@@ -59,6 +61,7 @@
    uint32_t n_slices;
    uint32_t n_ranges;
    uint32_t block_keys;
+   uint32_t n_items;
    const uint32_t* counters;
    double min_proportion[SILO_GPU_MAX_SCAN_BATCH];
    struct Range {
@@ -72,8 +75,8 @@
       uint32_t pos_end;
       uint32_t out_symbols;
       uint32_t key_from;
-      uint32_t first_block;
-      uint32_t blocks_per_slice;
+      uint32_t first_item;
+      uint32_t items_per_slice;
       uint32_t* counts[SILO_GPU_MAX_SCAN_BATCH];
    } ranges[ESCAPE_MAX_RANGES];
 };
@@ -94,8 +97,14 @@
    return (FILTERS * (ESCAPE_SLICE_WORDS32 + escapeWindow<FILTERS>()) + 3u * ESCAPE_GRANULES_PER_BLOCK + 4u + 64u) * static_cast<uint32_t>(sizeof(uint32_t));
 }
 
-template <int FILTERS>
-__global__ __launch_bounds__(ESCAPE_SLICE_THREADS, FILTERS <= 4 ? 8 : 4) void k_scan_escapes_sliced(const EscapeSliceArgs args, uint32_t n_filters) {
+struct EscapeBlockState {
+   uint32_t slice;
+   bool any_row;
+   bool zeroed;
+};
+
+template <int FILTERS, bool WALK>
+__device__ __forceinline__ void scanEscapeItem(const EscapeSliceArgs& args, const uint32_t n_filters, const uint32_t item, EscapeBlockState& kept) {
    constexpr uint32_t WINDOW = escapeWindow<FILTERS>();
    static_assert(ESCAPE_GRANULE_KEYS == ESCAPE_SLICE_THREADS * 4u, "a granule is one 16-byte load per thread of the block");
    extern __shared__ uint32_t s_filter[];
@@ -106,18 +115,22 @@
    uint32_t* s_nowhere = s_live + ESCAPE_GRANULES_PER_BLOCK + 4u;
    const uint32_t first_filter = blockIdx.z * FILTERS;
    uint32_t r = 0;
-   while (r + 1u < args.n_ranges && blockIdx.x >= args.ranges[r + 1u].first_block) {
+   while (r + 1u < args.n_ranges && item >= args.ranges[r + 1u].first_item) {
       ++r;
    }
    const EscapeSliceArgs::Range& range = args.ranges[r];
-   const uint32_t slice = (blockIdx.x - range.first_block) / range.blocks_per_slice;
-   const uint32_t share = (blockIdx.x - range.first_block) % range.blocks_per_slice;
+   const uint32_t slice = (item - range.first_item) / range.items_per_slice;
+   const uint32_t share = (item - range.first_item) % range.items_per_slice;
    const uint32_t out_symbols = range.out_symbols;
    const uint32_t* first = range.slice_first + static_cast<size_t>(slice) * (range.positions + 1u);
    const uint32_t key_begin = first[range.key_from];
    const uint32_t key_end = first[range.pos_end];
    const uint32_t share_begin = key_begin / ESCAPE_GRANULE_KEYS * ESCAPE_GRANULE_KEYS + share * args.block_keys;
    if (share_begin >= key_end) {
+      return;
+   }
+   const bool reload = !WALK || slice != kept.slice;
+   if (!reload && !kept.any_row) {
       return;
    }
    const uint32_t share_end = min(share_begin + args.block_keys, key_end);
@@ -167,6 +180,9 @@
       __syncthreads();
       n_live = liveGranule(ESCAPE_GRANULES_PER_BLOCK);
       if (n_live == 0) {
+         if constexpr (WALK) {
+            ldsBarrier();
+         }
          return;
       }
    }
@@ -183,7 +199,7 @@
 #pragma unroll
       for (uint32_t j = 0; j < ESCAPE_SLICE_WORDS32 / 4u / ESCAPE_SLICE_THREADS; ++j) {
          const uint32_t word = first_word + (j * ESCAPE_SLICE_THREADS + threadIdx.x) * 2u;
-         filter_part[f][j] = present && word < args.row_words ? *reinterpret_cast<const ulonglong2*>(filter + word) : make_ulonglong2(0, 0);
+         filter_part[f][j] = reload && present && word < args.row_words ? *reinterpret_cast<const ulonglong2*>(filter + word) : make_ulonglong2(0, 0);
       }
    }
    uint4 quad0 = prune ? loadKeys(0) : loadGranule(0);
@@ -194,39 +210,48 @@
    }
    constexpr bool BYTE_PER_ROW = FILTERS == 8;
    static_assert(ESCAPE_SLICE_WORDS32 / 4u / ESCAPE_SLICE_THREADS == 1u, "a thread holds one 16-byte part of a filter slice");
-#pragma unroll
-   for (int f = 0; f < FILTERS; ++f) {
-      for (uint32_t j = threadIdx.x * 4u; j < WINDOW; j += ESCAPE_SLICE_THREADS * 4u) {
-         *reinterpret_cast<uint4*>(s_count + f * WINDOW + j) = make_uint4(0, 0, 0, 0);
-      }
-      if constexpr (!BYTE_PER_ROW) {
-         *reinterpret_cast<ulonglong2*>(s_filter + f * ESCAPE_SLICE_WORDS32 + threadIdx.x * 4u) = filter_part[f][0];
-      }
-      any_bit |= filter_part[f][0].x | filter_part[f][0].y;
-   }
-   if constexpr (BYTE_PER_ROW) {
-#pragma unroll
-      for (uint32_t quarter = 0; quarter < 4; ++quarter) {
-         uint32_t bytes[8];
-#pragma unroll
-         for (uint32_t k = 0; k < 8; ++k) {
-            bytes[k] = 0;
-         }
-#pragma unroll
-         for (int f = 0; f < FILTERS; ++f) {
-            const uint64_t half = quarter < 2 ? filter_part[f][0].x : filter_part[f][0].y;
-            const uint32_t rows32 = static_cast<uint32_t>(half >> (32u * (quarter & 1u)));
+   if (!WALK || !kept.zeroed) {
+      for (uint32_t j = threadIdx.x * 4u; j < FILTERS * WINDOW; j += ESCAPE_SLICE_THREADS * 4u) {
+         *reinterpret_cast<uint4*>(s_count + j) = make_uint4(0, 0, 0, 0);
+      }
+      kept.zeroed = true;
+   }
+   if (!reload) {
+      ldsBarrier();
+   } else {
+#pragma unroll
+      for (int f = 0; f < FILTERS; ++f) {
+         if constexpr (!BYTE_PER_ROW) {
+            *reinterpret_cast<ulonglong2*>(s_filter + f * ESCAPE_SLICE_WORDS32 + threadIdx.x * 4u) = filter_part[f][0];
+         }
+         any_bit |= filter_part[f][0].x | filter_part[f][0].y;
+      }
+      if constexpr (BYTE_PER_ROW) {
+#pragma unroll
+         for (uint32_t quarter = 0; quarter < 4; ++quarter) {
+            uint32_t bytes[8];
 #pragma unroll
             for (uint32_t k = 0; k < 8; ++k) {
-               bytes[k] |= ((((rows32 >> (4u * k)) & 0xFu) * 0x00204081u) & 0x01010101u) << f;
-            }
-         }
-         uint32_t* out = s_filter + threadIdx.x * 32u + quarter * 8u;
-         *reinterpret_cast<uint4*>(out) = make_uint4(bytes[0], bytes[1], bytes[2], bytes[3]);
-         *reinterpret_cast<uint4*>(out + 4) = make_uint4(bytes[4], bytes[5], bytes[6], bytes[7]);
-      }
-   }
-   if (__syncthreads_or(any_bit != 0 ? 1 : 0) == 0) {
+               bytes[k] = 0;
+            }
+#pragma unroll
+            for (int f = 0; f < FILTERS; ++f) {
+               const uint64_t half = quarter < 2 ? filter_part[f][0].x : filter_part[f][0].y;
+               const uint32_t rows32 = static_cast<uint32_t>(half >> (32u * (quarter & 1u)));
+#pragma unroll
+               for (uint32_t k = 0; k < 8; ++k) {
+                  bytes[k] |= ((((rows32 >> (4u * k)) & 0xFu) * 0x00204081u) & 0x01010101u) << f;
+               }
+            }
+            uint32_t* out = s_filter + threadIdx.x * 32u + quarter * 8u;
+            *reinterpret_cast<uint4*>(out) = make_uint4(bytes[0], bytes[1], bytes[2], bytes[3]);
+            *reinterpret_cast<uint4*>(out + 4) = make_uint4(bytes[4], bytes[5], bytes[6], bytes[7]);
+         }
+      }
+      kept.any_row = __syncthreads_or(any_bit != 0 ? 1 : 0) != 0;
+      kept.slice = slice;
+   }
+   if (!kept.any_row) {
       return;
    }
    const uint32_t lane = __lane_id();
@@ -403,6 +428,18 @@
    flushChunk();
 }
 
+template <int FILTERS, bool WALK>
+__global__ __launch_bounds__(ESCAPE_SLICE_THREADS, (FILTERS <= 2 || (FILTERS <= 4 && !WALK)) ? 8 : 4) void k_scan_escapes_sliced(const EscapeSliceArgs args, uint32_t n_filters) {
+   EscapeBlockState kept{~0u, false, false};
+   if constexpr (!WALK) {
+      scanEscapeItem<FILTERS, false>(args, n_filters, blockIdx.x, kept);
+   } else {
+      for (uint32_t item = blockIdx.x; item < args.n_items; item += gridDim.x) {
+         scanEscapeItem<FILTERS, true>(args, n_filters, item, kept);
+      }
+   }
+}
+
 __global__ __launch_bounds__(256) void k_scan_escapes_overflow(
    const uint64_t* __restrict__ keys, uint32_t n_keys, const ScanBatchArgs batch, uint32_t pos_begin, uint32_t pos_end
 ) {
@@ -419,6 +456,67 @@
    }
 }
 
+static_assert(ESCAPE_PLAN_MAX_ENTRIES == ESCAPE_MAX_RANGES && ESCAPE_PLAN_GRANULE_KEYS == ESCAPE_GRANULE_KEYS && ESCAPE_PLAN_GRANULES_PER_ITEM == ESCAPE_GRANULES_PER_BLOCK,
+   "escape_item_plan.h repeats these constants so that it needs no HIP");
+
+template <int FILTERS, bool WALK>
+void launchEscapes(const dim3 grid, hipStream_t stream, const EscapeSliceArgs& args, uint32_t n_filters) {
+   k_scan_escapes_sliced<FILTERS, WALK><<<grid, ESCAPE_SLICE_THREADS, escapeLdsBytes<FILTERS>(), stream>>>(args, n_filters);
+}
+template <int FILTERS, bool WALK>
+hipError_t prepareEscapes(int* blocks_per_cu) {
+   if (const hipError_t e = hipFuncSetAttribute(reinterpret_cast<const void*>(k_scan_escapes_sliced<FILTERS, WALK>), hipFuncAttributeMaxDynamicSharedMemorySize, escapeLdsBytes<FILTERS>());
+       e != hipSuccess) {
+      return e;
+   }
+   return hipOccupancyMaxActiveBlocksPerMultiprocessor(blocks_per_cu, k_scan_escapes_sliced<FILTERS, WALK>, ESCAPE_SLICE_THREADS, escapeLdsBytes<FILTERS>());
+}
+template <bool WALK>
+void launchEscapes(uint32_t per_block, const dim3 grid, hipStream_t stream, const EscapeSliceArgs& args, uint32_t n_filters) {
+   switch (per_block) {
+      case 1: launchEscapes<1, WALK>(grid, stream, args, n_filters); break;
+      case 2: launchEscapes<2, WALK>(grid, stream, args, n_filters); break;
+      case 4: launchEscapes<4, WALK>(grid, stream, args, n_filters); break;
+      default: launchEscapes<8, WALK>(grid, stream, args, n_filters); break;
+   }
+}
+template <bool WALK>
+hipError_t prepareEscapes(uint32_t per_block, int* blocks_per_cu) {
+   switch (per_block) {
+      case 1: return prepareEscapes<1, WALK>(blocks_per_cu);
+      case 2: return prepareEscapes<2, WALK>(blocks_per_cu);
+      case 4: return prepareEscapes<4, WALK>(blocks_per_cu);
+      default: return prepareEscapes<8, WALK>(blocks_per_cu);
+   }
+}
+
+hipError_t escapePlaces(uint32_t per_block, bool walk, uint32_t* out) {
+   constexpr int MAX_DEVICES = 64;
+   static std::atomic<uint32_t> cached[MAX_DEVICES][4][2];
+   int device = 0;
+   if (const hipError_t e = hipGetDevice(&device); e != hipSuccess) {
+      return e;
+   }
+   if (device < 0 || device >= MAX_DEVICES) {
+      return hipErrorInvalidDevice;
+   }
+   std::atomic<uint32_t>& slot = cached[device][per_block == 1 ? 0 : (per_block == 2 ? 1 : (per_block == 4 ? 2 : 3))][walk ? 1 : 0];
+   *out = slot.load(std::memory_order_relaxed);
+   if (*out != 0) {
+      return hipSuccess;
+   }
+   int per_cu = 0, cus = 0;
+   if (const hipError_t e = walk ? prepareEscapes<true>(per_block, &per_cu) : prepareEscapes<false>(per_block, &per_cu); e != hipSuccess) {
+      return e;
+   }
+   if (const hipError_t e = hipDeviceGetAttribute(&cus, hipDeviceAttributeMultiprocessorCount, device); e != hipSuccess) {
+      return e;
+   }
+   *out = static_cast<uint32_t>(std::max(1, per_cu)) * static_cast<uint32_t>(std::max(1, cus));
+   slot.store(*out, std::memory_order_relaxed);
+   return hipSuccess;
+}
+
 ScanBatchArgs keyBatch(const ScanRange& range, const uint64_t* const* filters, uint32_t q_count) {
    ScanBatchArgs batch{};
    batch.out_symbols = range.seqstore->dev.n_scan;
@@ -430,6 +528,8 @@
 }
 
 namespace silo_gpu_detail {
+
+thread_local uint32_t g_last_escape_items = 0;
 
 int scanEscapes(
    const std::vector<ScanRange>& ranges, const uint64_t* const* filters, uint32_t q_count, hipStream_t hip_stream, const std::vector<ScanRange>* gaps,
@@ -443,34 +543,37 @@
       sliced.counters = pruning->counters;
    }
    uint32_t n_sliced = 0;
-   std::array<uint32_t, ESCAPE_MAX_RANGES> most_keys{};
+   std::array<EscapeEntryShape, ESCAPE_MAX_RANGES> shapes{};
    uint64_t total_keys = 0;
    bool end_entries = false;
    const auto launchSliced = [&]() -> int {
       if (n_sliced == 0) {
          return SILO_GPU_OK;
       }
-      static std::once_flag lds_once;
-      std::call_once(lds_once, [] {
-         (void)hipFuncSetAttribute(reinterpret_cast<const void*>(k_scan_escapes_sliced<1>), hipFuncAttributeMaxDynamicSharedMemorySize, escapeLdsBytes<1>());
-         (void)hipFuncSetAttribute(reinterpret_cast<const void*>(k_scan_escapes_sliced<2>), hipFuncAttributeMaxDynamicSharedMemorySize, escapeLdsBytes<2>());
-         (void)hipFuncSetAttribute(reinterpret_cast<const void*>(k_scan_escapes_sliced<4>), hipFuncAttributeMaxDynamicSharedMemorySize, escapeLdsBytes<4>());
-         (void)hipFuncSetAttribute(reinterpret_cast<const void*>(k_scan_escapes_sliced<8>), hipFuncAttributeMaxDynamicSharedMemorySize, escapeLdsBytes<8>());
-      });
       const uint32_t per_block = q_count <= 1 ? 1 : (q_count <= 2 ? 2 : (q_count <= 4 ? 4 : 8));
       const uint32_t passes = (q_count + per_block - 1) / per_block;
-      const uint64_t granules = (total_keys + ESCAPE_GRANULE_KEYS - 1) / ESCAPE_GRANULE_KEYS * passes;
-      const uint32_t block_granules = static_cast<uint32_t>(std::min<uint64_t>(ESCAPE_GRANULES_PER_BLOCK, std::max<uint64_t>(1, granules / 1280)));
-      const uint32_t block_keys = block_granules * ESCAPE_GRANULE_KEYS;
-      sliced.block_keys = block_keys;
+      const int knob = g_tune_escape_blocks.load();
+      uint32_t places = 0, walk_places = 0;
+      HIP_TRY(escapePlaces(per_block, false, &places));
+      if (knob != 0) {
+         HIP_TRY(escapePlaces(per_block, true, knob < 0 ? &places : &walk_places));
+      }
+      const EscapeItemPlan plan = planEscapeItems(shapes.data(), n_sliced, sliced.n_slices, passes, places, knob);
+      if (!plan.ok) {
+         return fail(SILO_GPU_ERR_INVALID_ARGUMENT, "scanEscapes: the launch has more items than the escape kernel numbers");
+      }
+      sliced.block_keys = plan.block_keys;
       sliced.n_ranges = n_sliced;
-      uint32_t blocks = 0;
+      sliced.n_items = plan.n_items;
+      std::array<EscapeSliceArgs::Range, ESCAPE_MAX_RANGES> as_added{};
+      std::copy_n(sliced.ranges, n_sliced, as_added.begin());
       for (uint32_t k = 0; k < n_sliced; ++k) {
-         sliced.ranges[k].first_block = blocks;
-         sliced.ranges[k].blocks_per_slice = std::max<uint32_t>(1, (most_keys[k] + block_keys - 1) / block_keys);
-         blocks += sliced.ranges[k].blocks_per_slice * sliced.n_slices;
-      }
-      const dim3 grid(blocks, 1, passes);
+         sliced.ranges[k] = as_added[plan.order[k]];
+         sliced.ranges[k].first_item = plan.first_item[k];
+         sliced.ranges[k].items_per_slice = plan.items_per_slice[k];
+      }
+      g_last_escape_items = plan.n_items;
+      const dim3 grid(plan.grid, 1, passes);
       char name[64];
       bool bounds = false;
       for (uint32_t k = 0; k < n_sliced; ++k) {
@@ -478,19 +581,18 @@
       }
       std::snprintf(name, sizeof(name), "k_scan_escapes_sliced<%u>%s%s", per_block, bounds ? ", pruning" : "", end_entries ? ", ends" : "");
       ScanLaunchTiming* timing = startLaunchTiming(
-         name, 0, total_keys * sizeof(uint32_t) * grid.z + static_cast<uint64_t>(grid.x) * q_count * ESCAPE_SLICE_WORDS32 * sizeof(uint32_t), q_count,
+         name, 0, total_keys * sizeof(uint32_t) * grid.z + static_cast<uint64_t>(plan.n_items) * q_count * ESCAPE_SLICE_WORDS32 * sizeof(uint32_t), q_count,
          grid.x * grid.z, hip_stream
       );
-      switch (per_block) {
-         case 1: k_scan_escapes_sliced<1><<<grid, ESCAPE_SLICE_THREADS, escapeLdsBytes<1>(), hip_stream>>>(sliced, q_count); break;
-         case 2: k_scan_escapes_sliced<2><<<grid, ESCAPE_SLICE_THREADS, escapeLdsBytes<2>(), hip_stream>>>(sliced, q_count); break;
-         case 4: k_scan_escapes_sliced<4><<<grid, ESCAPE_SLICE_THREADS, escapeLdsBytes<4>(), hip_stream>>>(sliced, q_count); break;
-         default: k_scan_escapes_sliced<8><<<grid, ESCAPE_SLICE_THREADS, escapeLdsBytes<8>(), hip_stream>>>(sliced, q_count); break;
+      if (plan.grid < plan.n_items) {
+         launchEscapes<true>(per_block, grid, hip_stream, sliced, q_count);
+      } else {
+         launchEscapes<false>(per_block, grid, hip_stream, sliced, q_count);
       }
       HIP_TRY(hipGetLastError());
       finishLaunchTiming(timing, hip_stream);
       n_sliced = 0;
-      most_keys.fill(0);
+      shapes.fill(EscapeEntryShape{});
       total_keys = 0;
       end_entries = false;
       return SILO_GPU_OK;
@@ -521,8 +623,10 @@
       for (uint32_t slice = 0; slice < n_slices; ++slice) {
          const uint32_t n = stream.slice_first[slice * stride + range.pos_end] - stream.slice_first[slice * stride + key_from];
          total_keys += n;
-         most_keys[n_sliced] = std::max(most_keys[n_sliced], n + ESCAPE_GRANULE_KEYS - 1u);
-      }
+         shapes[n_sliced].keys += n;
+         shapes[n_sliced].most_keys = std::max(shapes[n_sliced].most_keys, n + ESCAPE_GRANULE_KEYS - 1u);
+      }
+      shapes[n_sliced].prunable = heaviest != nullptr;
       ++n_sliced;
       return SILO_GPU_OK;
    };
diff --git a/lapis-silo_amd/csrc/store_internal.h b/lapis-silo_amd/csrc/store_internal.h
--- a/lapis-silo_amd/csrc/store_internal.h
+++ b/lapis-silo_amd/csrc/store_internal.h
@@ -23,6 +23,7 @@
 extern std::atomic<int> g_tune_prune_keys;
 extern std::atomic<int> g_tune_end_runs;
 extern std::atomic<int> g_tune_fused_select;
+extern std::atomic<int> g_tune_escape_blocks;
 extern std::atomic<int> g_tune_side_stream;
 extern std::atomic<int> g_tune_scan_timing;
 extern std::atomic<int> g_tune_missing_runs;
diff --git a/lapis-silo_amd/silo_amd/binding.py b/lapis-silo_amd/silo_amd/binding.py
--- a/lapis-silo_amd/silo_amd/binding.py
+++ b/lapis-silo_amd/silo_amd/binding.py
@@ -96,7 +96,7 @@
     "silo_gpu_malloc", "silo_gpu_memcpy_d2h", "silo_gpu_memcpy_h2d", "silo_gpu_stream_synchronize", "silo_gpu_stream_create", "silo_gpu_set_device", "silo_gpu_stream_destroy", "silo_gpu_store_plane",
     "silo_gpu_store_sparse_plane", "silo_gpu_filter_eval", "silo_gpu_filter_eval_batch", "silo_gpu_popcount", "silo_gpu_mutations_scan", "silo_gpu_mutations_scan_batch", "silo_gpu_mutations_scan_ranges", "silo_gpu_mutations_grouped", "silo_gpu_store_scan_planes", "silo_gpu_store_scan_escapes", "silo_gpu_store_scan_overflow_keys", "silo_gpu_store_scan_rows", "silo_gpu_store_scan_runs", "silo_gpu_row_slot_create", "silo_gpu_row_slot_destroy", "silo_gpu_mutations_select_to_slot", "silo_gpu_row_slot_wait", "silo_gpu_store_scan_sparse_keys", "silo_gpu_store_finalize_seqstore", "silo_gpu_store_build_pass", "silo_gpu_store_build_mode", "silo_gpu_store_memory_info", "silo_gpu_store_import_position", "silo_gpu_store_import_missing_rows",
     "silo_gpu_memset_async", "silo_gpu_event_create", "silo_gpu_event_record", "silo_gpu_event_elapsed_ms",
-    "silo_gpu_event_destroy", "silo_gpu_event_synchronize", "silo_gpu_host_alloc", "silo_gpu_host_free", "silo_gpu_memcpy_d2h_async", "silo_gpu_mutations_select", "silo_gpu_upload_bytes", "silo_gpu_upload_column", "silo_gpu_bitset_from_compare", "silo_gpu_group_count", "silo_gpu_group_count_hashed", "silo_gpu_reconstruct_sequences", "silo_gpu_bitset_from_pairs", "silo_gpu_count_pairs", "silo_gpu_count_slot_create", "silo_gpu_count_slot_destroy", "silo_gpu_filter_eval_count", "silo_gpu_count_slot_wait", "silo_gpu_tune", "silo_gpu_last_scan_kernel", "silo_gpu_scan_timings", "silo_gpu_stream_read_probe", "silo_gpu_last_error",
+    "silo_gpu_event_destroy", "silo_gpu_event_synchronize", "silo_gpu_host_alloc", "silo_gpu_host_free", "silo_gpu_memcpy_d2h_async", "silo_gpu_mutations_select", "silo_gpu_upload_bytes", "silo_gpu_upload_column", "silo_gpu_bitset_from_compare", "silo_gpu_group_count", "silo_gpu_group_count_hashed", "silo_gpu_reconstruct_sequences", "silo_gpu_bitset_from_pairs", "silo_gpu_count_pairs", "silo_gpu_count_slot_create", "silo_gpu_count_slot_destroy", "silo_gpu_filter_eval_count", "silo_gpu_count_slot_wait", "silo_gpu_tune", "silo_gpu_last_scan_kernel", "silo_gpu_last_escape_items", "silo_gpu_scan_timings", "silo_gpu_stream_read_probe", "silo_gpu_last_error",
     "silo_gpu_comm_unique_id", "silo_gpu_comm_create", "silo_gpu_comm_destroy", "silo_gpu_comm_rank", "silo_gpu_comm_world",
     "silo_gpu_allreduce_counts", "silo_gpu_broadcast_bytes",
     "silo_gpu_mutations_scan_select",
@@ -258,6 +258,8 @@
     lib.silo_gpu_event_destroy.restype = None
     lib.silo_gpu_tune.argtypes = [ctypes.c_int, ctypes.c_int]
     lib.silo_gpu_last_scan_kernel.restype = ctypes.c_char_p
+    lib.silo_gpu_last_escape_items.argtypes = []
+    lib.silo_gpu_last_escape_items.restype = ctypes.c_uint32
     lib.silo_gpu_store_build_pass.argtypes = [vp, ctypes.c_uint32, ctypes.c_int]
     lib.silo_gpu_store_build_pass.restype = ctypes.c_int
     lib.silo_gpu_store_build_mode.argtypes = [vp, ctypes.c_uint32]
```

Result: faster. 2000000 billion positions*sequences/s (median of 6 runs) (+7.9%).
